# tusen-ai/RangeDet

Measured on AMD Instinct MI355X. Metric: range-image frames/sec (64x2650, 8ch) at 1/2/4/8 GPU; Meta-Kernel HBM GB/s vs peak, higher is better.
Workload: dtype bf16

## Files before the change

### include/rangedet_hip.h

```cpp
#ifndef RANGEDET_HIP_H_
#define RANGEDET_HIP_H_
#include <stddef.h>
#include <stdint.h>

#ifdef __cplusplus
extern "C" {
#endif

#define RD_OK 0
#define RD_EINVAL (-1)
#define RD_ESHAPE (-2)
#define RD_EWORKSPACE (-3)
#define RD_EHIP (-4)

#define RD_F32 0
#define RD_BF16 1
#define RD_F16 2

#define RD_RELU_PRE 1
#define RD_ADD 2
#define RD_RELU_POST 4
#define RD_SCALE_FOLDED 8
#define RD_MFMA16 16

int rd_version(void);
const char* rd_last_error_string(void);

int rd_nchw_to_nhwc(const float* src, void* dst, int B, int C, int H, int W, int dst_cstride, int dst_coff,
                    int zero_pad, int dst_dtype, void* stream);
int rd_nhwc_to_nchw(const void* src, float* dst, int B, int C, int H, int W, int src_cstride, int src_coff,
                    int src_dtype, void* stream);

int rd_copy_rows(const void* src, long src_row_bytes, void* dst, long dst_row_bytes, long dst_offset_bytes, long bytes,
                 int rows, void* stream);

size_t rd_conv_packed_bytes(int ntaps, int cin, int cout, int dtype);
int rd_pack_conv_weight_host(const float* w_oihw_host, int cout, int cin, int kh, int kw, int dtype,
                             void* packed_host);
int rd_deconv_phase_taps(int kh, int kw, int stride_w, int pad_w, int phase);
int rd_pack_deconv_weight_host(const float* w_iohw_host, int cin, int cout, int kh, int kw, int stride_w,
                               int pad_w, int phase, int dtype, void* packed_host);
int rd_pack_deconv_weight_folded_host(const float* w_iohw_host, const float* fold_scale_host, int cin, int cout, int kh, int kw,
                                      int stride_w, int pad_w, int phase, int dtype, void* packed_host);

int rd_conv2d_bn_act(const void* x, int x_cstride, int x_coff, const void* w_packed, const float* scale,
                     const float* shift, const void* residual, int r_cstride, int r_coff, void* y,
                     int y_cstride, int y_coff, int B, int H, int Win, int cin, int cout, int kh, int kw,
                     int stride_w, int flags, int dtype, void* stream);
size_t rd_conv3x3_ex_packed_bytes(int cin, int cout, int stride_w, int x_cstride);
int rd_pack_conv3x3_ex_host(const float* w_oihw_host, const float* fold_scale_host, int cout, int cin, int stride_w,
                            int x_cstride, int dtype, void* packed_host);
int rd_pack_conv3x3_m16_host(const float* w_oihw_host, const float* fold_scale_host, int cout, int cin, int dtype, void* packed_host);
int rd_conv3x3_mfma16_ok(int cin, int cout, int stride_w, int W, int fused_output_conv);
size_t rd_conv1x1_sc_packed_bytes(int cin, int cout);
int rd_pack_conv1x1_sc_host(const float* w_oi_host, const float* fold_scale_host, int cout, int cin, int dtype,
                            void* packed_host);
int rd_conv3x3_bn_act_ex(const void* x, int x_cstride, int x_coff, const void* w_packed, const float* scale, const float* shift,
                         const void* residual, int r_cstride, int r_coff, const void* sc_x, int sc_cstride, int sc_coff,
                         int sc_cin, const void* sc_w_packed, void* y, int y_cstride, int y_coff, int B, int H, int Win, int cin,
                         int cout, int stride_w, int flags, int dtype, void* stream);
size_t rd_block64_packed_bytes(int cin);
int rd_pack_block64_host(const float* w1_oihw_host, const float* fold_scale1_host, const float* w2_oihw_host,
                         const float* fold_scale2_host, int cin, int dtype, void* packed_host);
int rd_block64_bn_act(const void* x, int x_cstride, int x_coff, int cin, const void* w_packed, const float* shift1, const float* shift2,
                      const void* sc_w_packed, void* y, int y_cstride, int y_coff, int B, int H, int W, int dtype, void* stream);
int rd_pack_block64_m16_host(const float* w1_oihw_host, const float* fold_scale1_host, const float* w2_oihw_host,
                             const float* fold_scale2_host, int dtype, void* packed_host);
int rd_pack_conv1x1_sc_m16_host(const float* w_oi_host, const float* fold_scale_host, int dtype, void* packed_host);
int rd_block64_m16_bn_act(const void* x, int x_cstride, int x_coff, const void* w_packed, const float* shift1, const float* shift2,
                          const void* sc_w_packed, void* y, int y_cstride, int y_coff, int B, int H, int W, int dtype, void* stream);

size_t rd_head_packed_bytes(void);
int rd_pack_head_weight_host(const float* w, int nout, int cin, int dtype, void* out_host);
size_t rd_head_m16_packed_bytes(void);
int rd_pack_head_weight_m16_host(const float* w, int nout, int cin, int dtype, void* out_host);
int rd_conv2d_bn_act_head_out(const void* x, int x_cstride, int x_coff, const void* w_packed, const float* scale,
                              const float* shift, int B, int H, int W, int cin, int flags, const void* head_w_packed,
                              const float* head_bias, float* out, long out_batch_stride, long n_off, int nout, int dtype,
                              void* stream);

int rd_conv3x3_bn_act_pair(const void* x0, int x0_coff, const void* w0_packed, const float* shift0, void* y0, int y0_coff,
                           const void* x1, int x1_coff, const void* w1_packed, const float* shift1, void* y1, int y1_coff,
                           int x_cstride, int y_cstride, int B, int H, int W, int cin, int flags, int dtype, void* stream);
int rd_conv2d_bn_act_head_out_pair(const void* x0, int x0_coff, const void* w0_packed, const float* shift0, const void* head_w0_packed,
                                   const float* head_bias0, float* out0, long out0_batch_stride, int nout0,
                                   const void* x1, int x1_coff, const void* w1_packed, const float* shift1, const void* head_w1_packed,
                                   const float* head_bias1, float* out1, long out1_batch_stride, int nout1,
                                   int x_cstride, long n_off, int B, int H, int W, int cin, int flags, int dtype, void* stream);

size_t rd_conv3x3_cat_packed_bytes(int cin1, int cin2, int cout);
int rd_pack_conv3x3_cat_host(const float* w, const float* fold_scale, int cout, int cin1, int cin2, int dtype, void* out_host);
int rd_conv3x3_bn_act_cat(const void* x1, int x1_cstride, int x1_coff, int cin1, const void* x2, int x2_cstride, int x2_coff, int cin2,
                          const void* w_packed, const float* shift, void* y, int y_cstride, int y_coff, int B, int H, int W, int cout,
                          int flags, int dtype, void* stream);

int rd_deconv2d_bn_act(const void* x, int x_cstride, int x_coff, const void* w_packed_phase,
                       const float* scale, const float* shift, const void* residual, int r_cstride,
                       int r_coff, void* y, int y_cstride, int y_coff, int B, int H, int Win, int cin,
                       int cout, int kh, int kw, int stride_w, int pad_w, int phase, int flags, int dtype,
                       void* stream);

int rd_deconv2d_all_phases_ok(int kh, int kw, int stride_w, int pad_w, int cout, int dtype);
int rd_deconv2d_bn_act_all(const void* x, int x_cstride, int x_coff, const void* w_packed_all, long w_phase_bytes,
                           const float* shift, const void* residual, int r_cstride, int r_coff, void* y, int y_cstride,
                           int y_coff, int B, int H, int Win, int cin, int cout, int kh, int kw, int stride_w, int pad_w,
                           int flags, int dtype, void* stream);

int rd_deconv2d_phase_pairs_ok(int kh, int kw, int stride_w, int pad_w, int cout, int dtype);
int rd_pack_deconv_phase_pair_host(const void* phase_a, const void* phase_b, int cin, int dtype, void* out);
int rd_deconv2d_bn_act_pairs(const void* x, int x_cstride, int x_coff, const void* w_packed_pairs, long w_pair_bytes,
                             const float* shift2, const void* residual, int r_cstride, int r_coff, void* y, int y_cstride,
                             int y_coff, int B, int H, int Win, int cin, int cout, int kh, int kw, int stride_w, int pad_w,
                             int flags, int dtype, void* stream);

int rd_head_out(const void* x, int x_cstride, int x_coff, const float* w, const float* bias, float* out,
                long out_batch_stride, long n_off, int B, int H, int W, int cin, int nout, int dtype,
                void* stream);

size_t rd_meta_packed_bytes(int dtype);
int rd_pack_meta_host(const float* w0, const float* b0, const float* w1, const float* b1, const float* s1,
                      const float* t1, const float* agg, const float* s2, const float* t2, int dtype,
                      void* packed_host);
int rd_meta_kernel_fwd(const void* data, int d_cstride, int d_coff, const float* coord_nchw,
                       const void* packed, void* y, int y_cstride, int y_coff, int B, int H, int W, int dtype,
                       void* stream);

size_t rd_sorted_foreground_workspace_bytes(long N, long k);
int rd_sorted_foreground(const float* cls_score, const float* bbox_delta, const float* pc, const float* mask,
                         int B, long N, long k, int D, int apply_sigmoid, float* out_score, float* out_delta,
                         float* out_pc, int* out_idx, void* ws, size_t ws_bytes, void* stream);

int rd_decode3d_bbox(const float* bbox_delta, const float* pc, float* out, int B, long N, int box_type,
                     int is_bin, void* stream);

size_t rd_score_filter_workspace_bytes(long n);
int rd_score_filter_dets(const float* scores, const float* boxes10, long n, float min_score, float* dets,
                         int* d_count, void* ws, size_t ws_bytes, void* stream);
int rd_score_filter_dets_batched(const float* scores, long scores_bstride, const float* boxes10, long boxes_bstride,
                                 long n, float min_score, float* dets, long dets_bstride, int* d_count, void* ws,
                                 size_t ws_bytes, int B, void* stream);

#define RD_WNMS_MAX_K 65536
#define RD_TIE_STABLE 0
#define RD_TIE_REFERENCE 1
#define RD_WNMS_DIAG_NO_SKIP 0x100
#define RD_WNMS_DIAG_TILE_W(n) (((n) & 0xff) << 16)
#define RD_WNMS_DIAG_MERGE_LDS(n) (((n) & 0x7f) << 24)
size_t rd_wnms_workspace_bytes(int Kcap);
int rd_wnms_4c(const float* dets, int Kcap, const int* d_count, const int* order, int tie_order, float thresh,
               float thresh_vote, int is3d, int hash_scale, float* out_dets, int* keep, int* d_nkeep, void* ws,
               size_t ws_bytes, void* stream);
int rd_wnms_4c_batched(const float* dets, long dets_bstride, int Kcap, const int* d_count, const int* order,
                       long order_bstride, int tie_order, float thresh, float thresh_vote, int is3d, int hash_scale,
                       float* out_dets, long out_bstride, int* keep, long keep_bstride, int* d_nkeep, void* ws,
                       size_t ws_bytes, int B, void* stream);
int rd_single_overlap(const float* dets_a, const float* dets_b, long n, int is3d, float* out, void* stream);
int rd_wnms_pair_skippable(const float* dets_a, const float* dets_b, long n, unsigned char* out, void* stream);

int rd_edge_atan2f(const float* y, const float* x, long n, float* out, void* stream);

int rd_wnms_order_host(const float* dets_host, int K, int* order_host);

int rd_dets12_to_8(const float* dets12, int Mcap, const int* d_count, float* out8, void* stream);
int rd_dets12_to_8_batched(const float* dets12, long dets12_bstride, int Mcap, const int* d_count, float* out8,
                           long out8_bstride, int B, void* stream);

int rd_rotated_iou_8pt(const float* boxes1, const float* boxes2, float* ious, long n1, long n2, void* stream);
int rd_batch_rotated_iou(const float* proposal, int p_stride, const float* gt_bbox, float* iou_map, int* argmax, int B, long N,
                         int n_gt, void* stream);
int rd_batch_rotated_iou_3d(const float* proposal, int p_stride, const float* gt_bbox7, float* iou_map, int* argmax, int B, long N,
                            int n_gt, void* stream);
int rd_rotated_iou_7(const float* boxes1, const float* boxes2, float* ious, long n1, long n2, void* stream);
int rd_batch_max_iou(const float* proposals, int p_stride, const float* gt8, float* out, long n, int n_gt,
                     void* stream);

size_t rd_nms3d_workspace_bytes(long N, int B);
int rd_gather_keep_scores(const float* score, long score_bstride, int k, const int* keep_idx, int max_keep, float* out, int B,
                          void* stream);
int rd_nms3d(const float* boxes, int B, long N, float iou_thres, int max_keep, int normal_iou, int* keep_idx,
             float* bbox_after_nms, void* ws, size_t ws_bytes, void* stream);

int rd_assign3d_v2(const float* pc, const float* bbox, const float* bbox_center, const float* bbox_radius, const float* mask,
                   const float* is_in_nlz, long N, int M, float max_x, float min_x, float max_y, float min_y, float max_z,
                   float min_z, float max_dist, int* out, void* stream);
size_t rd_get_point_num_workspace_bytes(void);
int rd_get_point_num(const float* bbox_inds, long N, float* out, void* ws, size_t ws_bytes, void* stream);

typedef struct {
  float clip_lo[7], clip_hi[7];
  float mean[8], sd[8];
  float interval_lo[3], interval_hi[3];
} rd_input_norm_t;
int rd_input_transform(const float* range_image, const float* pc_vehicle_frame, const float* inclination,
                       const rd_input_norm_t* norm_host, int B, int H, int W, int Hp, int Wp, float* input_data,
                       float* coord_s1, float* pc_s1, float* pc_s2, float* pc_s4, float* mask_s1, float* mask_s2,
                       float* mask_s4, void* stream);

typedef struct {
  float *input_data, *coord_s1;
  float *pc[3], *mask[3];
  float *reg_target[3], *reg_weight[3], *reg_normalize_weight[3], *cls_target[3];
  int* bbox3d_ind;
} rd_train_outputs_t;
size_t rd_train_transform_workspace_bytes(int B);
int rd_train_transform(const float* range_image, const float* pc_vehicle_frame, const float* inclination,
                       const rd_input_norm_t* norm_host, const float* gt_bbox_imu, const float* gt_bbox_center,
                       const float* gt_limits, const float* gt_bbox_csa, const int* num_gt_host, int Mmax, float radius,
                       float max_dist, const float* reg_weight_host, int B, int H, int W, int Hp, int Wp,
                       const rd_train_outputs_t* out_host, void* ws, size_t ws_bytes, void* stream);

#define RD_PROF_CONV 0
#define RD_PROF_META 1
#define RD_PROF_HEAD_OUT 2
#define RD_PROF_SORT 3
#define RD_PROF_DECODE 4
#define RD_PROF_WNMS 5
#define RD_PROF_LAYOUT 6
#define RD_PROF_CONV3 7
#define RD_PROF_BLOCK 8
#define RD_PROF_NKINDS 9
int rd_prof_enable(int on);
int rd_prof_reset(void);
int rd_prof_get(int kind, double* total_ms, long* launches);

#ifdef __cplusplus
}
#endif
#endif
```

### rangedet_amd/csrc/k_misc.h

```cpp
#pragma once
#include "rd_common.h"

namespace rd {

template <int DT>
__global__ __launch_bounds__(256) void nchw_to_nhwc_kernel(const float* __restrict__ src, void* __restrict__ dst_, int C,
                                                           long HW, int cs, int coff, int cpad, long total) {
  using E = Elem<DT>;
  typename E::T* dst = (typename E::T*)dst_;
  const int ctot = C + cpad;
  for (long i = blockIdx.x * 256L + threadIdx.x; i < total; i += (long)gridDim.x * 256) {
    long p = i % HW;
    long rest = i / HW;
    int c = (int)(rest % ctot);
    long b = rest / ctot;
    float v = c < C ? src[(b * C + c) * HW + p] : 0.f;
    dst[(b * HW + p) * cs + coff + c] = E::from_f32(v);
  }
}
template <int DT, int NSLOT>
__global__ __launch_bounds__(256) void nchw_to_nhwc_px_kernel(const float* __restrict__ src, void* __restrict__ dst_, int C,
                                                              long HW, int cs, int coff, long npix) {
  using E = Elem<DT>;
  typename E::T* dst = (typename E::T*)dst_;
  for (long i = blockIdx.x * 256L + threadIdx.x; i < npix; i += (long)gridDim.x * 256) {
    const long b = i / HW, p = i - b * HW;
    typename E::T v[NSLOT * E::CH];
#pragma unroll
    for (int c = 0; c < NSLOT * E::CH; ++c) v[c] = E::from_f32(c < C ? src[(b * C + c) * HW + p] : 0.f);
    Slot16 pk[NSLOT];
    memcpy(pk, v, sizeof(pk));
#pragma unroll
    for (int u = 0; u < NSLOT; ++u) *(Slot16*)(dst + i * cs + coff + u * E::CH) = pk[u];
  }
}
template <int DT>
__global__ __launch_bounds__(256) void nhwc_to_nchw_kernel(const void* __restrict__ src_, float* __restrict__ dst, int C,
                                                           long HW, int cs, int coff, long total) {
  using E = Elem<DT>;
  const typename E::T* src = (const typename E::T*)src_;
  for (long i = blockIdx.x * 256L + threadIdx.x; i < total; i += (long)gridDim.x * 256) {
    long p = i % HW;
    long rest = i / HW;
    int c = (int)(rest % C);
    long b = rest / C;
    dst[(b * C + c) * HW + p] = E::to_f32(src[(b * HW + p) * cs + coff + c]);
  }
}

template <int DT, int NOUT>
__global__ __launch_bounds__(256) void head_out_kernel(const void* __restrict__ x_, int cs, int coff,
                                                       const float* __restrict__ w, const float* __restrict__ bias,
                                                       float* __restrict__ out, long out_bs, long n_off, long HW,
                                                       int cin) {
  using E = Elem<DT>;
  using T = typename E::T;
  __shared__ float wl[8 * 128];
  const T* x = (const T*)x_ + (size_t)blockIdx.y * HW * cs;
  for (int i = threadIdx.x; i < NOUT * cin; i += 256) wl[i] = w[i];
  __syncthreads();
  const int sub = threadIdx.x & 7;
  const int per = cin >> 3;
  const long npix_iter = (long)gridDim.x * 32;
  for (long p0 = blockIdx.x * 32L; p0 < HW; p0 += npix_iter) {
    long p = p0 + (threadIdx.x >> 3);
    float acc[NOUT];
#pragma unroll
    for (int o = 0; o < NOUT; ++o) acc[o] = 0.f;
    if (p < HW) {
      const T* px = x + p * cs + coff + sub * per;
      if ((per % E::CH) == 0) {
        for (int c0 = 0; c0 < per; c0 += E::CH) {
          const Slot16 raw = *(const Slot16*)(px + c0);
          T el[E::CH];
          memcpy(el, &raw, 16);
#pragma unroll
          for (int e = 0; e < E::CH; ++e) {
            const float v = E::to_f32(el[e]);
#pragma unroll
            for (int o = 0; o < NOUT; ++o) acc[o] += v * wl[o * cin + sub * per + c0 + e];
          }
        }
      } else {
        for (int c = 0; c < per; ++c) {
          float v = E::to_f32(px[c]);
#pragma unroll
          for (int o = 0; o < NOUT; ++o) acc[o] += v * wl[o * cin + sub * per + c];
        }
      }
    }
#pragma unroll
    for (int o = 0; o < NOUT; ++o) {
      acc[o] += __shfl_xor(acc[o], 1);
      acc[o] += __shfl_xor(acc[o], 2);
      acc[o] += __shfl_xor(acc[o], 4);
    }
    if (p < HW && sub == 0) {
      float* o_ = out + (size_t)blockIdx.y * out_bs + (n_off + p) * NOUT;
#pragma unroll
      for (int o = 0; o < NOUT; ++o) o_[o] = acc[o] + bias[o];
    }
  }
}

template <int NOUT, int DT = RD_BF16>
__global__ __launch_bounds__(256) void head_out_mfma_kernel(const bf16_t* __restrict__ x, int cs, int coff,
                                                            const float* __restrict__ w, const float* __restrict__ bias,
                                                            float* __restrict__ out, long out_bs, long n_off, long HW,
                                                            int cin) {
  __shared__ __attribute__((aligned(16))) unsigned char lds[4 * 8192];
  const int lane = threadIdx.x & 63, m = lane & 31, hi = lane >> 5, wv = threadIdx.x >> 6;
  unsigned char* img = lds + wv * 8192;
  const int nks = cin >> 4, nsl = cin >> 3;
  x += (size_t)blockIdx.y * HW * cs + coff;
  out += (size_t)blockIdx.y * out_bs + n_off * NOUT;
  s16x8 wh[8], wl[8];
#pragma unroll
  for (int ks = 0; ks < 8; ++ks) {
    unsigned short h[8], l[8];
#pragma unroll
    for (int j = 0; j < 8; ++j) {
      const float v = (m < NOUT && ks < nks) ? w[m * cin + ks * 16 + hi * 8 + j] : 0.f;
      h[j] = H16<DT>::from_f32(v);
      l[j] = H16<DT>::from_f32(v - H16<DT>::to_f32(h[j]));
    }
    memcpy(&wh[ks], h, 16);
    memcpy(&wl[ks], l, 16);
  }
  float bs[4];
#pragma unroll
  for (int r = 0; r < 4; ++r) bs[r] = 4 * hi + r < NOUT ? bias[4 * hi + r] : 0.f;
  const long ntile = (HW + 31) / 32;
  const long wave0 = (long)blockIdx.x * 4 + wv, nwave = (long)gridDim.x * 4;
  const int lp = lane >> 4, ls = lane & 15;
  auto load = [&](long tile, Slot16 (&v)[8]) {
#pragma unroll
    for (int it = 0; it < 8; ++it) {
      const long p = min(tile * 32 + it * 4 + lp, HW - 1);
      v[it] = ls < nsl ? *(const Slot16*)(x + p * cs + ls * 8) : Slot16{0u, 0u, 0u, 0u};
    }
  };
  Slot16 cur[8], nxt[8];
  if (wave0 < ntile) load(wave0, cur);
  for (long tile = wave0; tile < ntile; tile += nwave) {
    const bool more = tile + nwave < ntile;
    if (more) load(tile + nwave, nxt);
#pragma unroll
    for (int it = 0; it < 8; ++it) {
      const int pr = it * 4 + lp;
      *(Slot16*)(img + pr * 256 + ((ls ^ (pr & 15)) << 4)) = cur[it];
    }
    __builtin_amdgcn_wave_barrier();
    f32x16 acc;
#pragma unroll
    for (int r = 0; r < 16; ++r) acc[r] = 0.f;
#pragma unroll
    for (int ks = 0; ks < 8; ++ks) {
      const s16x8 b = *(const s16x8*)(img + m * 256 + (((2 * ks + hi) ^ (m & 15)) << 4));
      acc = H16<DT>::mfma(wl[ks], b, acc);
      acc = H16<DT>::mfma(wh[ks], b, acc);
    }
    __builtin_amdgcn_wave_barrier();
    const long p = tile * 32 + m;
    if (p < HW) {
      float* o = out + p * NOUT + 4 * hi;
#pragma unroll
      for (int r = 0; r < 4; ++r)
        if (4 * hi + r < NOUT) o[r] = acc[r] + bs[r];
    }
    if (more) {
#pragma unroll
      for (int it = 0; it < 8; ++it) cur[it] = nxt[it];
    }
  }
}

__global__ __launch_bounds__(256) void decode3d_kernel(const float* __restrict__ delta, const float* __restrict__ pc,
                                                       float* __restrict__ out, long n, int box_type, int is_bin) {
  long idx = blockIdx.x * 256L + threadIdx.x;
  if (idx >= n) return;
  const float* d = delta + idx * box_type;
  float pc_x = pc[idx * 3 + 0], pc_y = pc[idx * 3 + 1], pc_z = pc[idx * 3 + 2];
  float az = atan2f(pc_y, pc_x);
  float ca = cosf(az), sa = sinf(az);
  float dx, dy, width, length, height, z0, yaw_l;
  if (is_bin) {
    dx = d[0];
    dy = d[1];
    width = expf(d[3]);
    length = expf(d[4]);
    height = expf(d[5]);
    float cz = pc_z + d[2];
    z0 = (float)((double)cz - (double)height / 2.0);
    yaw_l = d[6] + az;
  } else {
    dx = d[0] * fabsf(d[0]);
    dy = d[1] * fabsf(d[1]);
    width = expf(d[2]);
    length = expf(d[3]);
    height = expf(d[7]);
    z0 = d[6];
    yaw_l = atan2f(d[5], d[4]) + az;
  }
  float dxl = dx * ca - dy * sa;
  float dyl = dx * sa + dy * ca;
  float cx = pc_x + dxl, cy = pc_y + dyl;
  float sy = sinf(yaw_l), cyw = cosf(yaw_l);
  float hl = (float)(0.5 * (double)length), hw = (float)(0.5 * (double)width);
  float hx[4] = {hl, -hl, -hl, hl};
  float hy[4] = {-hw, -hw, hw, hw};
  float* o = out + idx * 10;
#pragma unroll
  for (int k = 0; k < 4; ++k) {
    o[2 * k] = (hx[k] * cyw - hy[k] * sy) + cx;
    o[2 * k + 1] = (hx[k] * sy + hy[k] * cyw) + cy;
  }
  o[8] = z0;
  o[9] = z0 + height;
}

__global__ __launch_bounds__(256) void filter_count_kernel(const float* __restrict__ scores, long n, float thr,
                                                           int* __restrict__ blk_cnt, long sc_bs, long blk_bs) {
  scores += blockIdx.y * sc_bs;
  blk_cnt += blockIdx.y * blk_bs;
  long i = blockIdx.x * 256L + threadIdx.x;
  int p = (i < n) && (scores[i] > thr);
  unsigned long long m = __ballot(p);
  __shared__ int wc[4];
  if ((threadIdx.x & 63) == 0) wc[threadIdx.x >> 6] = __popcll(m);
  __syncthreads();
  if (threadIdx.x == 0) blk_cnt[blockIdx.x] = wc[0] + wc[1] + wc[2] + wc[3];
}
__global__ __launch_bounds__(256) void filter_scan_kernel(int* __restrict__ blk_cnt, int nblk, int* __restrict__ total,
                                                          long blk_bs) {
  blk_cnt += blockIdx.x * blk_bs;
  total += blockIdx.x;
  __shared__ int part[256];
  __shared__ int carry;
  if (threadIdx.x == 0) carry = 0;
  __syncthreads();
  for (int base = 0; base < nblk; base += 256) {
    int i = base + threadIdx.x;
    int v = i < nblk ? blk_cnt[i] : 0;
    part[threadIdx.x] = v;
    __syncthreads();
    for (int off = 1; off < 256; off <<= 1) {
      int t = threadIdx.x >= off ? part[threadIdx.x - off] : 0;
      __syncthreads();
      part[threadIdx.x] += t;
      __syncthreads();
    }
    int incl = part[threadIdx.x];
    if (i < nblk) blk_cnt[i] = carry + incl - v;
    __syncthreads();
    if (threadIdx.x == 255) carry += incl;
    __syncthreads();
  }
  if (threadIdx.x == 0) *total = carry;
}
__global__ __launch_bounds__(256) void filter_scatter_kernel(const float* __restrict__ scores,
                                                             const float* __restrict__ boxes10, long n, float thr,
                                                             const int* __restrict__ blk_off, float* __restrict__ dets,
                                                             long sc_bs, long box_bs, long blk_bs, long dets_bs) {
  scores += blockIdx.y * sc_bs;
  boxes10 += blockIdx.y * box_bs;
  blk_off += blockIdx.y * blk_bs;
  dets += blockIdx.y * dets_bs;
  long i = blockIdx.x * 256L + threadIdx.x;
  int p = (i < n) && (scores[i] > thr);
  unsigned long long m = __ballot(p);
  __shared__ int wc[4];
  const int wv = threadIdx.x >> 6, ln = threadIdx.x & 63;
  if (ln == 0) wc[wv] = __popcll(m);
  __syncthreads();
  int off = blk_off[blockIdx.x];
  for (int w = 0; w < wv; ++w) off += wc[w];
  if (p) {
    int pos = off + __popcll(m & ((1ull << ln) - 1ull));
    const float* b = boxes10 + i * 10;
    float* d = dets + (size_t)pos * 12;
#pragma unroll
    for (int k = 0; k < 8; ++k) d[k] = b[k];
    d[8] = fdlibm_atan2f(b[1] - b[3], b[0] - b[2]);
    d[9] = b[8];
    d[10] = b[9] - b[8];
    d[11] = scores[i];
  }
}

__global__ __launch_bounds__(256) void dets12_to_8_kernel(const float* __restrict__ d12, int cap, const int* __restrict__ d_count,
                                                          float* __restrict__ o8, long d12_bs, long o8_bs) {
  d12 += blockIdx.y * d12_bs;
  o8 += blockIdx.y * o8_bs;
  int i = blockIdx.x * 256 + threadIdx.x;
  int n = d_count ? min(d_count[blockIdx.y], cap) : cap;
  if (i >= n) return;
  const float* d = d12 + (size_t)i * 12;
  float* o = o8 + (size_t)i * 8;
  o[0] = (d[0] + d[2] + d[4] + d[6]) / 4.f;
  o[1] = (d[1] + d[3] + d[5] + d[7]) / 4.f;
  o[2] = d[9] + d[10] / 2.f;
  float ax = d[2] - d[0], ay = d[3] - d[1];
  float bx = d[2] - d[4], by = d[3] - d[5];
  o[3] = sqrtf(ax * ax + ay * ay);
  o[4] = sqrtf(bx * bx + by * by);
  o[5] = d[10];
  o[6] = d[8];
  o[7] = d[11];
}

__global__ __launch_bounds__(256) void gather_keep_scores_kernel(const float* __restrict__ score, long score_bs, int k,
                                                                 const int* __restrict__ keep, int mk, float* __restrict__ out) {
  const int i = blockIdx.x * 256 + threadIdx.x;
  if (i >= mk) return;
  const int q = keep[(size_t)blockIdx.y * mk + i];
  out[(size_t)blockIdx.y * mk + i] = (q >= 0 && q < k) ? score[blockIdx.y * score_bs + q] : -__builtin_inff();
}

}
```

### rangedet_amd/csrc/k_sort.h

```cpp
#pragma once
#include "rd_common.h"

namespace rd {

constexpr int SORT_TILE = 2048;

__device__ __forceinline__ unsigned desc_key(float f) {
  unsigned u = __float_as_uint(f);
  unsigned asc = u ^ ((u >> 31) ? 0xFFFFFFFFu : 0x80000000u);
  return ~asc;
}
__device__ __forceinline__ float key_to_float(unsigned key) {
  unsigned asc = ~key;
  unsigned u = (asc >> 31) ? (asc ^ 0x80000000u) : ~asc;
  return __uint_as_float(u);
}

__global__ __launch_bounds__(256) void sort_keygen_kernel(const float* __restrict__ score, const float* __restrict__ mask,
                                                          long N, int apply_sigmoid, unsigned* __restrict__ keys,
                                                          unsigned* __restrict__ idx, long ws_stride) {
  long i = blockIdx.x * 256L + threadIdx.x;
  if (i >= N) return;
  const long b = blockIdx.y;
  float s = score[b * N + i];
  if (apply_sigmoid) s = 1.0f / (1.0f + expf(-s));
  if (mask) s = s * mask[b * N + i];
  keys[b * ws_stride + i] = desc_key(s);
  idx[b * ws_stride + i] = (unsigned)i;
}
__global__ __launch_bounds__(256) void sort_keygen_dets_kernel(const float* __restrict__ dets, int cap,
                                                               const int* __restrict__ d_count, unsigned* __restrict__ keys,
                                                               unsigned* __restrict__ idx) {
  int i = blockIdx.x * 256 + threadIdx.x;
  if (i >= cap) return;
  int n = d_count ? min(*d_count, cap) : cap;
  keys[i] = i < n ? desc_key(dets[(size_t)i * 12 + 11]) : 0xFFFFFFFFu;
  idx[i] = (unsigned)i;
}

__global__ __launch_bounds__(256) void sort_hist_kernel(const unsigned* __restrict__ keys, long N, int shift,
                                                        unsigned* __restrict__ hist, unsigned* __restrict__ tot,
                                                        long ws_stride, const unsigned* __restrict__ d_n) {
  if (d_n) N = min(N, (long)d_n[blockIdx.y * ws_stride]);
  keys += blockIdx.y * ws_stride;
  hist += blockIdx.y * ws_stride;
  tot += blockIdx.y * ws_stride;
  __shared__ unsigned h[256];
  h[threadIdx.x] = 0;
  __syncthreads();
  long base = (long)blockIdx.x * SORT_TILE;
  for (int r = 0; r < SORT_TILE / 256; ++r) {
    long i = base + r * 256 + threadIdx.x;
    if (i < N) atomicAdd(&h[(keys[i] >> shift) & 255u], 1u);
  }
  __syncthreads();
  unsigned v = h[threadIdx.x];
  hist[(size_t)blockIdx.x * 256 + threadIdx.x] = v;
  if (v) atomicAdd(&tot[threadIdx.x], v);
}

__global__ __launch_bounds__(256) void sort_scatter_kernel(const unsigned* __restrict__ keys_in,
                                                           const unsigned* __restrict__ idx_in, long N, int shift,
                                                           const unsigned* __restrict__ hist,
                                                           const unsigned* __restrict__ tot,
                                                           unsigned* __restrict__ keys_out, unsigned* __restrict__ idx_out,
                                                           long ws_stride, const unsigned* __restrict__ d_n) {
  if (d_n) {
    N = min(N, (long)d_n[blockIdx.y * ws_stride]);
    if ((long)blockIdx.x * SORT_TILE >= N) return;
  }
  {
    const long o = blockIdx.y * ws_stride;
    keys_in += o; idx_in += o; hist += o; tot += o; keys_out += o; idx_out += o;
  }
  __shared__ unsigned wcnt[4][256];
  __shared__ unsigned gbase[256];
  __shared__ unsigned scan[256];
  const int tid = threadIdx.x, lane = tid & 63, wv = tid >> 6;
  for (int w = 0; w < 4; ++w) wcnt[w][tid] = 0;
  {
    unsigned t = tot[tid];
    scan[tid] = t;
    __syncthreads();
    for (int off = 1; off < 256; off <<= 1) {
      unsigned a = tid >= off ? scan[tid - off] : 0u;
      __syncthreads();
      scan[tid] += a;
      __syncthreads();
    }
    unsigned before = 0;
    for (unsigned b = 0; b < blockIdx.x; ++b) before += hist[(size_t)b * 256 + tid];
    gbase[tid] = scan[tid] - t + before;
  }
  __syncthreads();

  unsigned key[8], id[8], pos[8];
  const long base = (long)blockIdx.x * SORT_TILE + wv * 512;
  const unsigned long long lt = (1ull << lane) - 1ull;
#pragma unroll
  for (int r = 0; r < 8; ++r) {
    long i = base + r * 64 + lane;
    bool valid = i < N;
    key[r] = valid ? keys_in[i] : 0xFFFFFFFFu;
    id[r] = valid ? idx_in[i] : 0u;
    unsigned d = (key[r] >> shift) & 255u;
    unsigned long long peers = __ballot(valid);
#pragma unroll
    for (int bit = 0; bit < 8; ++bit) {
      unsigned long long bm = __ballot(valid && ((d >> bit) & 1u));
      peers &= ((d >> bit) & 1u) ? bm : ~bm;
    }
    unsigned rank = __popcll(peers & lt), cnt = __popcll(peers);
    unsigned prev = wcnt[wv][d];
    pos[r] = prev + rank;
    __builtin_amdgcn_wave_barrier();
    if (valid && rank == 0) wcnt[wv][d] = prev + cnt;
    __builtin_amdgcn_wave_barrier();
  }
  __syncthreads();
  {
    unsigned c0 = wcnt[0][tid], c1 = wcnt[1][tid], c2 = wcnt[2][tid];
    wcnt[0][tid] = 0;
    wcnt[1][tid] = c0;
    wcnt[2][tid] = c0 + c1;
    wcnt[3][tid] = c0 + c1 + c2;
  }
  __syncthreads();
#pragma unroll
  for (int r = 0; r < 8; ++r) {
    long i = base + r * 64 + lane;
    if (i < N) {
      unsigned d = (key[r] >> shift) & 255u;
      unsigned dst = gbase[d] + wcnt[wv][d] + pos[r];
      keys_out[dst] = key[r];
      idx_out[dst] = id[r];
    }
  }
}

__global__ __launch_bounds__(256) void sort_gather_kernel(const unsigned* __restrict__ keys, const unsigned* __restrict__ idx,
                                                          long k, int D, const float* __restrict__ delta,
                                                          const float* __restrict__ pc, float* __restrict__ out_score,
                                                          float* __restrict__ out_delta, float* __restrict__ out_pc,
                                                          int* __restrict__ out_idx, long ws_stride, long N) {
  long i = blockIdx.x * 256L + threadIdx.x;
  if (i >= k) return;
  {
    const long b = blockIdx.y;
    keys += b * ws_stride; idx += b * ws_stride;
    delta += b * N * D; pc += b * N * 3;
    out_score += b * k; out_delta += b * k * D; out_pc += b * k * 3;
    if (out_idx) out_idx += b * k;
  }
  unsigned j = idx[i];
  out_score[i] = key_to_float(keys[i]);
  for (int c = 0; c < D; ++c) out_delta[i * D + c] = delta[(size_t)j * D + c];
  out_pc[i * 3 + 0] = pc[(size_t)j * 3 + 0];
  out_pc[i * 3 + 1] = pc[(size_t)j * 3 + 1];
  out_pc[i * 3 + 2] = pc[(size_t)j * 3 + 2];
  if (out_idx) out_idx[i] = (int)j;
}

constexpr int SEL_BINS = 4096, SEL_SHIFT = 20;
__global__ __launch_bounds__(256) void select_hist_kernel(const unsigned* __restrict__ keys, long N, unsigned* __restrict__ h12,
                                                          long ws_stride) {
  keys += blockIdx.y * ws_stride; h12 += blockIdx.y * ws_stride;
  __shared__ unsigned h[SEL_BINS];
  for (int i = threadIdx.x; i < SEL_BINS; i += 256) h[i] = 0;
  __syncthreads();
  const long base = (long)blockIdx.x * SORT_TILE;
  for (int r = 0; r < SORT_TILE / 256; ++r) {
    const long i = base + r * 256 + threadIdx.x;
    if (i < N) atomicAdd(&h[keys[i] >> SEL_SHIFT], 1u);
  }
  __syncthreads();
  for (int i = threadIdx.x; i < SEL_BINS; i += 256)
    if (h[i]) atomicAdd(&h12[i], h[i]);
}
__global__ __launch_bounds__(256) void select_thresh_kernel(const unsigned* __restrict__ h12, long k, unsigned* __restrict__ sel,
                                                            long ws_stride) {
  h12 += blockIdx.y * ws_stride; sel += blockIdx.y * ws_stride;
  __shared__ unsigned part[256];
  const int tid = threadIdx.x;
  unsigned loc[SEL_BINS / 256], sum = 0;
#pragma unroll
  for (int j = 0; j < SEL_BINS / 256; ++j) { loc[j] = h12[tid * (SEL_BINS / 256) + j]; sum += loc[j]; }
  part[tid] = sum;
  __syncthreads();
  for (int off = 1; off < 256; off <<= 1) {
    const unsigned v = tid >= off ? part[tid - off] : 0u;
    __syncthreads();
    part[tid] += v;
    __syncthreads();
  }
  unsigned before = part[tid] - sum;
  if (tid == 255 && (k == 0 || part[255] < (unsigned)k)) { sel[0] = SEL_BINS - 1; sel[1] = part[255]; }
  if (before < (unsigned)k && before + sum >= (unsigned)k) {
#pragma unroll
    for (int j = 0; j < SEL_BINS / 256; ++j) {
      if (before < (unsigned)k && before + loc[j] >= (unsigned)k) { sel[0] = tid * (SEL_BINS / 256) + j; sel[1] = before + loc[j]; }
      before += loc[j];
    }
  }
}
__global__ __launch_bounds__(256) void select_count_kernel(const unsigned* __restrict__ keys, long N, const unsigned* __restrict__ sel,
                                                           unsigned* __restrict__ cnt, long ws_stride) {
  keys += blockIdx.y * ws_stride; sel += blockIdx.y * ws_stride; cnt += blockIdx.y * ws_stride;
  const unsigned T = sel[0];
  __shared__ unsigned c;
  if (threadIdx.x == 0) c = 0;
  __syncthreads();
  const long base = (long)blockIdx.x * SORT_TILE;
  unsigned mine = 0;
  for (int r = 0; r < SORT_TILE / 256; ++r) {
    const long i = base + r * 256 + threadIdx.x;
    if (i < N && (keys[i] >> SEL_SHIFT) <= T) ++mine;
  }
  if (mine) atomicAdd(&c, mine);
  __syncthreads();
  if (threadIdx.x == 0) cnt[blockIdx.x] = c;
}
__global__ __launch_bounds__(256) void select_compact_kernel(const unsigned* __restrict__ keys_in, const unsigned* __restrict__ idx_in,
                                                             long N, const unsigned* __restrict__ sel,
                                                             const unsigned* __restrict__ cnt, unsigned* __restrict__ keys_out,
                                                             unsigned* __restrict__ idx_out, long ws_stride) {
  {
    const long o = blockIdx.y * ws_stride;
    keys_in += o; idx_in += o; sel += o; cnt += o; keys_out += o; idx_out += o;
  }
  const unsigned T = sel[0];
  __shared__ unsigned wcnt[4][8], sbase;
  const int tid = threadIdx.x, lane = tid & 63, wv = tid >> 6;
  if (tid == 0) {
    unsigned b = 0;
    for (unsigned j = 0; j < blockIdx.x; ++j) b += cnt[j];
    sbase = b;
  }
  const long base = (long)blockIdx.x * SORT_TILE + wv * 512;
  unsigned key[8], id[8];
  unsigned long long m[8];
#pragma unroll
  for (int r = 0; r < 8; ++r) {
    const long i = base + r * 64 + lane;
    const bool valid = i < N;
    key[r] = valid ? keys_in[i] : 0xFFFFFFFFu;
    id[r] = valid ? idx_in[i] : 0u;
    m[r] = __ballot(valid && (key[r] >> SEL_SHIFT) <= T);
    if (lane == 0) wcnt[wv][r] = (unsigned)__popcll(m[r]);
  }
  __syncthreads();
  unsigned off = sbase;
  for (int w = 0; w < wv; ++w)
#pragma unroll
    for (int r = 0; r < 8; ++r) off += wcnt[w][r];
#pragma unroll
  for (int r = 0; r < 8; ++r) {
    if ((m[r] >> lane) & 1ull) {
      const unsigned dst = off + (unsigned)__popcll(m[r] & ((1ull << lane) - 1ull));
      keys_out[dst] = key[r];
      idx_out[dst] = id[r];
    }
    off += (unsigned)__popcll(m[r]);
  }
}

struct SortWs {
  unsigned *keysA, *keysB, *idxA, *idxB, *hist, *tot, *h12, *cnt, *sel;
  int nblk;
};
inline size_t sort_ws_bytes(long N) {
  long nblk = (N + SORT_TILE - 1) / SORT_TILE;
  return (size_t)(4 * N + nblk * 256 + 4 * 256 + SEL_BINS + nblk + 64) * 4 + 256;
}
inline SortWs sort_ws_carve(void* ws, long N) {
  SortWs s;
  s.nblk = (int)((N + SORT_TILE - 1) / SORT_TILE);
  unsigned* p = (unsigned*)ws;
  s.keysA = p; p += N;
  s.keysB = p; p += N;
  s.idxA = p; p += N;
  s.idxB = p; p += N;
  s.hist = p; p += (size_t)s.nblk * 256;
  s.tot = p; p += 4 * 256;
  s.h12 = p; p += SEL_BINS;
  s.cnt = p; p += s.nblk;
  s.sel = p;
  return s;
}
inline int sort_clear(const SortWs& s, hipStream_t st, int nb, long ws_stride, bool with_h12) {
  const size_t bytes = (size_t)(4 * 256 + (with_h12 ? SEL_BINS : 0)) * 4;
  const hipError_t e = nb > 1 ? hipMemset2DAsync(s.tot, (size_t)ws_stride * 4, 0, bytes, nb, st) : hipMemsetAsync(s.tot, 0, bytes, st);
  return e == hipSuccess ? RD_OK : fail(RD_EHIP, "sort: memset");
}
inline int radix_sort_pairs(const SortWs& s, long N, hipStream_t st, int nb = 1, long ws_stride = 0, const unsigned* d_n = nullptr,
                            bool cleared = false) {
  if (!cleared) { int rc = sort_clear(s, st, nb, ws_stride, false); if (rc != RD_OK) return rc; }
  unsigned *ki = s.keysA, *ko = s.keysB, *ii = s.idxA, *io = s.idxB;
  for (int pass = 0; pass < 4; ++pass) {
    hipLaunchKernelGGL(sort_hist_kernel, dim3(s.nblk, nb), dim3(256), 0, st, ki, N, pass * 8, s.hist, s.tot + pass * 256,
                       ws_stride, d_n);
    hipLaunchKernelGGL(sort_scatter_kernel, dim3(s.nblk, nb), dim3(256), 0, st, ki, ii, N, pass * 8, s.hist,
                       s.tot + pass * 256, ko, io, ws_stride, d_n);
    std::swap(ki, ko);
    std::swap(ii, io);
  }
  return check_launch("radix_sort_pairs");
}

inline int radix_topk_pairs(const SortWs& s, long N, long k, hipStream_t st, int nb, long ws_stride, unsigned** rk, unsigned** ri) {
  const bool off = dev_switches().sort_no_select;
  *rk = s.keysA; *ri = s.idxA;
  RD_REQUIRE(k > 0 && k <= N, RD_ESHAPE, "top-k: k %ld of N %ld", k, N);
  if (off || 2 * k > N) return radix_sort_pairs(s, N, st, nb, ws_stride);
  { int rc = sort_clear(s, st, nb, ws_stride, true); if (rc != RD_OK) return rc; }
  hipLaunchKernelGGL(select_hist_kernel, dim3(s.nblk, nb), dim3(256), 0, st, s.keysA, N, s.h12, ws_stride);
  hipLaunchKernelGGL(select_thresh_kernel, dim3(1, nb), dim3(256), 0, st, s.h12, k, s.sel, ws_stride);
  hipLaunchKernelGGL(select_count_kernel, dim3(s.nblk, nb), dim3(256), 0, st, s.keysA, N, s.sel, s.cnt, ws_stride);
  hipLaunchKernelGGL(select_compact_kernel, dim3(s.nblk, nb), dim3(256), 0, st, s.keysA, s.idxA, N, s.sel, s.cnt, s.keysB, s.idxB,
                     ws_stride);
  SortWs v = s;
  v.keysA = s.keysB; v.keysB = s.keysA; v.idxA = s.idxB; v.idxB = s.idxA;
  *rk = s.keysB; *ri = s.idxB;
  return radix_sort_pairs(v, N, st, nb, ws_stride, s.sel + 1, true);
}

}
```

### rangedet_amd/csrc/rd_api.hip

```cpp
#include "k_conv1.h"
#include "k_block.h"
#include "k_assign.h"
#include "k_input.h"
#include "k_target.h"
#include "k_nms3d.h"
#include "k_meta.h"
#include "k_misc.h"
#include "k_riou.h"
#include "k_sort.h"
#include "k_wnms.h"

#include <algorithm>
#include <string>
#include <numeric>

using namespace rd;

namespace rd {
inline size_t align256(size_t v) { return (v + 255) & ~(size_t)255; }
inline size_t wnms_ws_bytes(int cap) {
  const size_t nw = (size_t)(cap + 63) / 64;
  return align256((size_t)cap * PREP_F * 4) + 3 * align256((size_t)cap * nw * 8) + 4 * align256((size_t)cap * 4) +
         align256(((size_t)cap + 2) * 8 + 3 * ((size_t)cap / 32 + 2) * 4) + align256(nw * 8) + 256 + align256(sort_ws_bytes(cap)) + 256;
}
// ... 478 lines not shown
}

int rd_deconv2d_all_phases_ok(int kh, int kw, int stride_w, int pad_w, int cout, int dtype) {
  if (!is_h16(dtype) || kh != 3 || stride_w < 2 || stride_w > 8 || !conv3_phases_eligible(cout, RD_SCALE_FOLDED)) return 0;
  if (kw - 2 * pad_w != stride_w) return 0;
  for (int p = 0; p < stride_w; ++p)
    if (!deconv_tap_set(deconv_taps_sorted(kh, kw, stride_w, pad_w, p))) return 0;
  return 1;
}
int rd_deconv2d_bn_act_all(const void* x, int x_cstride, int x_coff, const void* w_packed_all, long w_phase_bytes,
                           const float* shift, const void* residual, int r_cstride, int r_coff, void* y, int y_cstride,
                           int y_coff, int B, int H, int Win, int cin, int cout, int kh, int kw, int stride_w, int pad_w,
                           int flags, int dtype, void* stream) {
  RD_REQUIRE(x && w_packed_all && y, RD_EINVAL, "deconv2d_all: null pointer");
  RD_REQUIRE(is_h16(dtype), RD_EINVAL, "deconv2d_all: dtype %d (RD_BF16 or RD_F16)", dtype);
  RD_REQUIRE(flags & RD_SCALE_FOLDED, RD_EINVAL, "deconv2d_all: needs RD_SCALE_FOLDED weights (rd_pack_deconv_weight_folded_host)");
  RD_REQUIRE(!((flags & RD_ADD) && !residual), RD_EINVAL, "deconv2d_all: RD_ADD without residual");
  RD_REQUIRE(B > 0 && H > 0 && Win > 0 && cin > 0, RD_ESHAPE, "deconv2d_all: shape");
  RD_REQUIRE(y_coff >= 0 && y_coff + cout <= y_cstride, RD_ESHAPE, "deconv2d_all: y channels exceed stride");
  RD_REQUIRE(x_cstride % 8 == 0 && x_coff % 8 == 0 && x_coff + cin_slots(cin, RD_BF16) * 8 <= x_cstride, RD_ESHAPE, "deconv2d_all: x channel stride/offset");
  RD_REQUIRE(rd_deconv2d_all_phases_ok(kh, kw, stride_w, pad_w, cout, dtype), RD_ESHAPE,
             "deconv2d_all: kernel (%d,%d) stride %d pad %d cout %d is not a set of two-column 3x2 phases (use rd_deconv2d_bn_act per phase)",
             kh, kw, stride_w, pad_w, cout);
  RD_REQUIRE(w_phase_bytes >= (long)conv_packed_bytes(6, cin, cout, RD_BF16) && w_phase_bytes % 16 == 0, RD_EINVAL, "deconv2d_all: w_phase_bytes");
  allow_conv_lds();
  Conv3Phases ph;
  ph.nph = stride_w; ph.ts_mask = 0; ph.y_pc = y_cstride; ph.r_pc = r_cstride; ph.w_pb = w_phase_bytes;
  for (int p = 0; p < stride_w; ++p)
    if (deconv_tap_set(deconv_taps_sorted(kh, kw, stride_w, pad_w, p)) == 2) ph.ts_mask |= 1 << p;
  return launch_conv3(x, x_cstride, x_coff, w_packed_all, nullptr, shift, residual, r_cstride * stride_w, r_coff, y, y_cstride * stride_w,
                      y_coff, B, H, Win, cin, cout, flags, 1, (hipStream_t)stream, 3, nullptr, dtype, nullptr, &ph);
}

int rd_deconv2d_phase_pairs_ok(int kh, int kw, int stride_w, int pad_w, int cout, int dtype) {
  if (!rd_deconv2d_all_phases_ok(kh, kw, stride_w, pad_w, cout, dtype) || cout != 64 || stride_w % 2) return 0;
  if (!rd_deconv2d_all_phases_ok(kh, kw, stride_w, pad_w, 128, dtype)) return 0;
  for (int p = 0; p < stride_w; p += 2)
    if (deconv_tap_set(deconv_taps_sorted(kh, kw, stride_w, pad_w, p)) != deconv_tap_set(deconv_taps_sorted(kh, kw, stride_w, pad_w, p + 1))) return 0;
  return 1;
}
int rd_pack_deconv_phase_pair_host(const void* phase_a, const void* phase_b, int cin, int dtype, void* out) {
  RD_REQUIRE(phase_a && phase_b && out, RD_EINVAL, "pack_deconv_pair: null pointer");
  RD_REQUIRE(is_h16(dtype) && cin > 0, RD_EINVAL, "pack_deconv_pair: dtype %d / cin %d", dtype, cin);
  const size_t body = conv_packed_body_bytes(6, cin, 64, RD_BF16), blocks = body / 2048;
  for (size_t i = 0; i < blocks; ++i) {
    memcpy((unsigned char*)out + i * 4096, (const unsigned char*)phase_a + i * 2048, 2048);
    memcpy((unsigned char*)out + i * 4096 + 2048, (const unsigned char*)phase_b + i * 2048, 2048);
  }
  memset((unsigned char*)out + 2 * body, 0, 2 * RD_CONV_TAIL);
  return RD_OK;
}
int rd_deconv2d_bn_act_pairs(const void* x, int x_cstride, int x_coff, const void* w_packed_pairs, long w_pair_bytes,
                             const float* shift2, const void* residual, int r_cstride, int r_coff, void* y, int y_cstride,
                             int y_coff, int B, int H, int Win, int cin, int cout, int kh, int kw, int stride_w, int pad_w,
                             int flags, int dtype, void* stream) {
  RD_REQUIRE(x && w_packed_pairs && y && shift2, RD_EINVAL, "deconv2d_pairs: null pointer");
  RD_REQUIRE(is_h16(dtype), RD_EINVAL, "deconv2d_pairs: dtype %d (RD_BF16 or RD_F16)", dtype);
  RD_REQUIRE(flags & RD_SCALE_FOLDED, RD_EINVAL, "deconv2d_pairs: needs RD_SCALE_FOLDED weights (rd_pack_deconv_weight_folded_host)");
  RD_REQUIRE(!((flags & RD_ADD) && !residual), RD_EINVAL, "deconv2d_pairs: RD_ADD without residual");
  RD_REQUIRE(B > 0 && H > 0 && Win > 0 && cin > 0, RD_ESHAPE, "deconv2d_pairs: shape");
  RD_REQUIRE(x_cstride % 8 == 0 && x_coff % 8 == 0 && x_coff + cin_slots(cin, RD_BF16) * 8 <= x_cstride, RD_ESHAPE, "deconv2d_pairs: x channel stride/offset");
  RD_REQUIRE(rd_deconv2d_phase_pairs_ok(kh, kw, stride_w, pad_w, cout, dtype), RD_ESHAPE,
             "deconv2d_pairs: kernel (%d,%d) stride %d pad %d cout %d has no phase pairs (use rd_deconv2d_bn_act_all)", kh, kw, stride_w, pad_w, cout);
  RD_REQUIRE(y_cstride == cout && y_coff == 0 && (!residual || (r_cstride == cout && r_coff == 0)), RD_ESHAPE,
             "deconv2d_pairs: the output / residual must be dense %d-channel tensors (two phases are one 128-channel write)", cout);
  RD_REQUIRE(w_pair_bytes >= (long)conv_packed_bytes(6, cin, 2 * cout, RD_BF16) && w_pair_bytes % 16 == 0, RD_EINVAL, "deconv2d_pairs: w_pair_bytes");
  allow_conv_lds();
  Conv3Phases ph;
  ph.nph = stride_w / 2; ph.ts_mask = 0; ph.y_pc = 2 * cout; ph.r_pc = 2 * cout; ph.w_pb = w_pair_bytes;
  for (int p = 0; p < stride_w; p += 2)
    if (deconv_tap_set(deconv_taps_sorted(kh, kw, stride_w, pad_w, p)) == 2) ph.ts_mask |= 1 << (p / 2);
  return launch_conv3(x, x_cstride, x_coff, w_packed_pairs, nullptr, shift2, residual, r_cstride * stride_w, r_coff, y, y_cstride * stride_w,
                      y_coff, B, H, Win, cin, 2 * cout, flags, 1, (hipStream_t)stream, 3, nullptr, dtype, nullptr, &ph);
}

int rd_head_out(const void* x, int x_cstride, int x_coff, const float* w, const float* bias, float* out,
                long out_batch_stride, long n_off, int B, int H, int W, int cin, int nout, int dtype, void* stream) {
  RD_REQUIRE(x && w && bias && out, RD_EINVAL, "head_out: null pointer");
  RD_REQUIRE(cin % 8 == 0 && cin <= 128 && cin > 0, RD_ESHAPE, "head_out: cin %d (multiple of 8, <= 128)", cin);
  RD_REQUIRE(nout == 1 || nout == 7 || nout == 8, RD_ESHAPE, "head_out: nout %d not in {1,7,8}", nout);
  RD_REQUIRE(dtype == RD_F32 || is_h16(dtype), RD_EINVAL, "head_out: dtype");
  hipStream_t st = (hipStream_t)stream;
  const long HW = (long)H * W;
  dim3 grid((unsigned)std::min<long>((HW + 31) / 32, 4096), B);
  ProfScope ps(RD_PROF_HEAD_OUT, st);
  if (is_h16(dtype) && nout > 1 && cin % 16 == 0 && x_cstride % 8 == 0 && x_coff % 8 == 0) {
    dim3 g2((unsigned)std::min<long>((HW + 127) / 128, 2048), B);
#define RD_HOM(NO, DT_) hipLaunchKernelGGL((head_out_mfma_kernel<NO, DT_>), g2, dim3(256), 0, st, (const bf16_t*)x, x_cstride, x_coff, w, bias, out, out_batch_stride, n_off, HW, cin)
    if (dtype == RD_F16) { if (nout == 7) RD_HOM(7, RD_F16); else RD_HOM(8, RD_F16); }
    else { if (nout == 7) RD_HOM(7, RD_BF16); else RD_HOM(8, RD_BF16); }
#undef RD_HOM
    return check_launch("head_out");
  }
#define RD_HO(DT, NO) hipLaunchKernelGGL((head_out_kernel<DT, NO>), grid, dim3(256), 0, st, x, x_cstride, x_coff, w, bias, out, out_batch_stride, n_off, HW, cin)
  if (dtype == RD_BF16) { if (nout == 1) RD_HO(RD_BF16, 1); else if (nout == 7) RD_HO(RD_BF16, 7); else RD_HO(RD_BF16, 8); }
  else if (dtype == RD_F16) { if (nout == 1) RD_HO(RD_F16, 1); else if (nout == 7) RD_HO(RD_F16, 7); else RD_HO(RD_F16, 8); }
  else { if (nout == 1) RD_HO(RD_F32, 1); else if (nout == 7) RD_HO(RD_F32, 7); else RD_HO(RD_F32, 8); }
#undef RD_HO
  return check_launch("head_out");
}

size_t rd_meta_packed_bytes(int dtype) { return meta_layout(dtype).total; }
int rd_pack_meta_host(const float* w0, const float* b0, const float* w1, const float* b1, const float* s1,
                      const float* t1, const float* agg, const float* s2, const float* t2, int dtype, void* out) {
  RD_REQUIRE(w0 && b0 && w1 && b1 && s1 && t1 && agg && s2 && t2 && out, RD_EINVAL, "pack_meta: null pointer");
  RD_REQUIRE(dtype == RD_F32 || is_h16(dtype), RD_EINVAL, "pack_meta: dtype");
  pack_meta(w0, b0, w1, b1, s1, t1, agg, s2, t2, dtype, out);
  return RD_OK;
}
int rd_meta_kernel_fwd(const void* data, int d_cstride, int d_coff, const float* coord_nchw, const void* packed,
                       void* y, int y_cstride, int y_coff, int B, int H, int W, int dtype, void* stream) {
  RD_REQUIRE(data && coord_nchw && packed && y, RD_EINVAL, "meta_kernel: null pointer");
  RD_REQUIRE(B > 0 && H > 0 && W > 0, RD_ESHAPE, "meta_kernel: empty shape");
  RD_REQUIRE(dtype == RD_F32 || is_h16(dtype), RD_EINVAL, "meta_kernel: dtype");
  const int ch = ch_per_slot(dtype);
  RD_REQUIRE(d_cstride % ch == 0 && d_coff % ch == 0 && y_cstride % ch == 0 && y_coff % ch == 0, RD_ESHAPE,
             "meta_kernel: channel strides/offsets must be 16-byte multiples");
  RD_REQUIRE(d_coff + 64 <= d_cstride && y_coff + 64 <= y_cstride, RD_ESHAPE, "meta_kernel: needs 64 channels");
  hipStream_t st = (hipStream_t)stream;
  MetaArgs a;
  a.data = data; a.d_cs = d_cstride; a.d_co = d_coff; a.coord = coord_nchw; a.packed = (const unsigned char*)packed;
  a.y = y; a.y_cs = y_cstride; a.y_co = y_coff; a.B = B; a.H = H; a.W = W;
  constexpr int WAVES = 8;
  a.tiles_h = (H + WAVES - 1) / WAVES;
  a.tiles_w = (W + 31) / 32;
  a.ntiles = B * a.tiles_h * a.tiles_w;
  a.r0 = 0; a.m0 = a.m1 = a.m2 = 0;
  const size_t consts = 9 * 64 * 4 * 2 + 1024;
  ProfScope ps(RD_PROF_META, st);
  if (is_h16(dtype)) {
    const size_t lds = meta_layout(dtype).wbytes + consts + (size_t)(WAVES + 2) * 34 * 128 + 4096;
    static std::atomic<unsigned long long> seen{0};
    once_per_device(seen, [] { allow_big_lds(meta16_kernel<WAVES, RD_BF16>); allow_big_lds(meta16_kernel<WAVES, RD_F16>); });
    const dim3 mgrid(std::min(a.ntiles, conv_num_cus())), mblock(WAVES * 64);
    const int strips = a.tiles_w * B;
    a.r0 = dev_switches().conv_xcd && strips % 8 == 0 ? 8 : strips;
    RD_REQUIRE((unsigned long long)a.ntiles * (unsigned)std::max(a.r0, std::max(a.tiles_h, a.tiles_w)) < (1ull << 32), RD_ESHAPE,
               "meta_kernel: %d tiles exceed the range of the tile decode", a.ntiles);
    a.m0 = meta_magic(a.r0); a.m1 = meta_magic(a.tiles_h); a.m2 = meta_magic(a.tiles_w);
    RD_REQUIRE((long)H * W < (1l << 23) && (long)H * W * d_cstride < (1l << 31) && W < (1 << 23) && d_cstride < (1 << 23), RD_ESHAPE,
               "meta_kernel: image of %d x %d pixels x %d channels exceeds the 32-bit halo offsets", H, W, d_cstride);
    if (dtype == RD_F16) hipLaunchKernelGGL((meta16_kernel<WAVES, RD_F16>), mgrid, mblock, lds, st, a);
    else hipLaunchKernelGGL((meta16_kernel<WAVES, RD_BF16>), mgrid, mblock, lds, st, a);
  } else {
    const size_t lds = consts + (size_t)(WAVES + 2) * 34 * 256;
    static std::atomic<unsigned long long> seen32{0};
    once_per_device(seen32, [] { allow_big_lds(meta_kernel<RD_F32, WAVES>); });
    hipLaunchKernelGGL((meta_kernel<RD_F32, WAVES>), dim3(std::min(a.ntiles, 512)), dim3(WAVES * 64), lds, st, a);
  }
  return check_launch("meta_kernel");
}

size_t rd_sorted_foreground_workspace_bytes(long N, long k) { (void)k; return (sort_ws_bytes(N) + 256 + 255) & ~(size_t)255; }
int rd_sorted_foreground(const float* cls_score, const float* bbox_delta, const float* pc, const float* mask, int B,
                         long N, long k, int D, int apply_sigmoid, float* out_score, float* out_delta, float* out_pc,
                         int* out_idx, void* ws, size_t ws_bytes, void* stream) {
  RD_REQUIRE(cls_score && bbox_delta && pc && out_score && out_delta && out_pc && ws, RD_EINVAL, "sorted_foreground: null pointer");
  RD_REQUIRE(B > 0 && N > 0 && k > 0 && D > 0, RD_ESHAPE, "sorted_foreground: empty shape");
  RD_REQUIRE(N >= k, RD_ESHAPE, "sorted_foreground: N (%ld) < num_fgs (%ld)", N, k);
  RD_REQUIRE(N < (1L << 31), RD_ESHAPE, "sorted_foreground: N too large");
  RD_REQUIRE(ws_bytes >= rd_sorted_foreground_workspace_bytes(N, k), RD_EWORKSPACE, "sorted_foreground: workspace %zu < %zu",
             ws_bytes, rd_sorted_foreground_workspace_bytes(N, k));
  hipStream_t st = (hipStream_t)stream;
  void* wsa = (void*)(((uintptr_t)ws + 255) & ~(uintptr_t)255);
  SortWs s = sort_ws_carve(wsa, N);
  ProfScope ps(RD_PROF_SORT, st);
  const size_t per = rd_sorted_foreground_workspace_bytes(N, k);
  const bool wide = ws_bytes >= per * (size_t)B;
  const long stride = wide ? (long)(per / 4) : 0;
  const int nb = wide ? B : 1;
  for (int b0 = 0; b0 < B; b0 += nb) {
    hipLaunchKernelGGL(sort_keygen_kernel, dim3((unsigned)((N + 255) / 256), nb), dim3(256), 0, st, cls_score + (size_t)b0 * N,
                       mask ? mask + (size_t)b0 * N : nullptr, N, apply_sigmoid, s.keysA, s.idxA, stride);
    unsigned *rk, *ri;
    int rc = radix_topk_pairs(s, N, k, st, nb, stride, &rk, &ri);
    if (rc != RD_OK) return rc;
    hipLaunchKernelGGL(sort_gather_kernel, dim3((unsigned)((k + 255) / 256), nb), dim3(256), 0, st, rk, ri, k, D,
                       bbox_delta + (size_t)b0 * N * D, pc + (size_t)b0 * N * 3, out_score + (size_t)b0 * k,
                       out_delta + (size_t)b0 * k * D, out_pc + (size_t)b0 * k * 3, out_idx ? out_idx + (size_t)b0 * k : nullptr,
                       stride, N);
  }
  return check_launch("sorted_foreground");
}

int rd_decode3d_bbox(const float* bbox_delta, const float* pc, float* out, int B, long N, int box_type, int is_bin,
                     void* stream) {
  RD_REQUIRE(bbox_delta && pc && out, RD_EINVAL, "decode3d: null pointer");
  RD_REQUIRE(B > 0 && N > 0, RD_ESHAPE, "decode3d: empty shape");
  RD_REQUIRE((is_bin && box_type == 7) || (!is_bin && box_type == 8), RD_ESHAPE,
             "decode3d: box_type %d with is_bin=%d (8 for regular, 7 for bin)", box_type, is_bin);
  hipStream_t st = (hipStream_t)stream;
  const long n = (long)B * N;
  ProfScope ps(RD_PROF_DECODE, st);
  hipLaunchKernelGGL(decode3d_kernel, dim3((unsigned)((n + 255) / 256)), dim3(256), 0, st, bbox_delta, pc, out, n, box_type, is_bin);
  return check_launch("decode3d");
}

size_t rd_score_filter_workspace_bytes(long n) { return (size_t)((n + 255) / 256 + 8) * 4 + 256; }
int rd_score_filter_dets_batched(const float* scores, long scores_bstride, const float* boxes10, long boxes_bstride,
                                 long n, float min_score, float* dets, long dets_bstride, int* d_count, void* ws,
                                 size_t ws_bytes, int B, void* stream) {
  RD_REQUIRE(scores && boxes10 && dets && d_count && ws, RD_EINVAL, "score_filter: null pointer");
  RD_REQUIRE(n > 0 && B > 0, RD_ESHAPE, "score_filter: empty input");
  const size_t per = rd_score_filter_workspace_bytes(n);
  RD_REQUIRE(ws_bytes >= per * (size_t)B, RD_EWORKSPACE, "score_filter: workspace %zu < %zu", ws_bytes, per * (size_t)B);
  hipStream_t st = (hipStream_t)stream;
  int* blk = (int*)(((uintptr_t)ws + 255) & ~(uintptr_t)255);
  const int nblk = (int)((n + 255) / 256);
  const long blk_bs = nblk + 8;
  ProfScope ps(RD_PROF_WNMS, st);
  hipLaunchKernelGGL(filter_count_kernel, dim3(nblk, B), dim3(256), 0, st, scores, n, min_score, blk, scores_bstride, blk_bs);
  hipLaunchKernelGGL(filter_scan_kernel, dim3(B), dim3(256), 0, st, blk, nblk, d_count, blk_bs);
  hipLaunchKernelGGL(filter_scatter_kernel, dim3(nblk, B), dim3(256), 0, st, scores, boxes10, n, min_score, blk, dets,
                     scores_bstride, boxes_bstride, blk_bs, dets_bstride);
  return check_launch("score_filter");
}
int rd_score_filter_dets(const float* scores, const float* boxes10, long n, float min_score, float* dets, int* d_count,
                         void* ws, size_t ws_bytes, void* stream) {
  return rd_score_filter_dets_batched(scores, 0, boxes10, 0, n, min_score, dets, 0, d_count, ws, ws_bytes, 1, stream);
}

size_t rd_wnms_workspace_bytes(int Kcap) { return Kcap > 0 ? wnms_ws_bytes(Kcap) : 0; }
int rd_wnms_4c_batched(const float* dets, long dets_bstride, int Kcap, const int* d_count, const int* order,
                       long order_bstride, int tie_order, float thresh, float thresh_vote, int is3d, int hash_scale,
                       float* out_dets, long out_bstride, int* keep, long keep_bstride, int* d_nkeep, void* ws,
                       size_t ws_bytes, int B, void* stream) {
  RD_REQUIRE(dets && out_dets && keep && d_nkeep && ws, RD_EINVAL, "wnms_4c: null pointer");
  RD_REQUIRE(Kcap > 0 && Kcap <= RD_WNMS_MAX_K, RD_ESHAPE, "wnms_4c: Kcap %d not in [1, %d]", Kcap, RD_WNMS_MAX_K);
  RD_REQUIRE(B > 0, RD_ESHAPE, "wnms_4c: batch %d", B);
  const int diag = tie_order & ~0xff;
  tie_order &= 0xff;
  RD_REQUIRE(tie_order == RD_TIE_STABLE || tie_order == RD_TIE_REFERENCE, RD_EINVAL, "wnms_4c: tie_order %d", tie_order);
  RD_REQUIRE(!(diag & ~(RD_WNMS_DIAG_NO_SKIP | (0xff << 16) | (0x7f << 24))), RD_EINVAL, "wnms_4c: unknown diagnostic bits 0x%x", diag);
  const size_t per = rd_wnms_workspace_bytes(Kcap);
  RD_REQUIRE(ws_bytes >= per * (size_t)B, RD_EWORKSPACE, "wnms_4c: workspace %zu < %zu", ws_bytes, per * (size_t)B);
  RD_REQUIRE(order || B == 1 || tie_order == RD_TIE_REFERENCE, RD_EINVAL,
             "wnms_4c: the batched call needs an explicit processing order or RD_TIE_REFERENCE");
  hipStream_t st = (hipStream_t)stream;
  static std::atomic<unsigned long long> seen_lds{0};
  once_per_device(seen_lds, [] {
    allow_big_lds(wnms_tie_order_kernel); allow_big_lds(wnms_scan_kernel); allow_big_lds(wnms_scan4_kernel); allow_big_lds(wnms_merge_kernel);
  });
  WnmsWs w = wnms_ws_carve(ws, Kcap);
  ProfScope ps(RD_PROF_WNMS, st);
  WnmsBatch bs;
  bs.dets = dets_bstride; bs.order = order_bstride; bs.prep = (long)(per / 4); bs.words = (long)(per / 8);
  bs.ints = (long)(per / 4); bs.keep = keep_bstride; bs.out = out_bstride;
  const int* ord = order;
  if (!ord && tie_order == RD_TIE_REFERENCE) {
    const size_t lds = TIE_STACK_BYTES + (Kcap <= TIE_LDS_K ? (size_t)Kcap * 8 + 3 * ((size_t)Kcap / 32 + 2) * 4 : 0);
    hipLaunchKernelGGL(wnms_tie_order_kernel, dim3(1, 1, B), dim3(256), lds, st, dets, Kcap, d_count, w.order, bs, (long)(per / 4),
                       w.scratch);
    ord = w.order;
    bs.order = (long)(per / 4);
  } else if (!ord) {
    void* swa = (void*)(((uintptr_t)w.sort_ws + 255) & ~(uintptr_t)255);
    SortWs s = sort_ws_carve(swa, Kcap);
    hipLaunchKernelGGL(sort_keygen_dets_kernel, dim3((Kcap + 255) / 256), dim3(256), 0, st, dets, Kcap, d_count, s.keysA, s.idxA);
    int rc = radix_sort_pairs(s, Kcap, st);
    if (rc != RD_OK) return rc;
    if (hipMemcpyAsync(w.order, s.idxA, (size_t)Kcap * 4, hipMemcpyDeviceToDevice, st) != hipSuccess)
      return rd::fail(RD_EHIP, "wnms_4c: order copy");
    ord = w.order;
    bs.order = 0;
  }
  const int nb = (Kcap + 63) / 64;
  hipLaunchKernelGGL(wnms_prep_kernel, dim3((Kcap + 255) / 256, 1, B), dim3(256), 0, st, dets, ord, Kcap, d_count, w.prep, bs,
                     (float)hash_scale, w.novf);
  const int e_tw = (diag >> 16) & 0xff, e_ml = (diag >> 24) & 0x7f;
  const int tile_w = std::min(w.nwcap, e_tw ? std::max(1, e_tw) : 256);
  const size_t scan_lds = ((size_t)w.nwcap + (size_t)64 * tile_w) * 8;
  const int R1 = 256, nb1 = R1 / 64;
  const bool one_round = dev_switches().wnms_one_round;
  const bool two = Kcap >= 4 * R1 && !one_round;
  const int ct = dev_switches().wnms_ct == 32 ? 32 : dev_switches().wnms_ct == 16 ? 16 : 8;
  const int pgrid = std::min(2048, std::max(64, nb * (64 / ct) * std::min(nb, 16)));
  const int allow_skip = thresh >= 1e-3f && thresh_vote >= 1e-3f && !is3d && !dev_switches().wnms_no_skip && !(diag & RD_WNMS_DIAG_NO_SKIP);
  auto pairs = [&](const int* rows, const int* nrows, const unsigned long long* supp, int rb_end) {
    auto k = dev_switches().wnms_bal ? (ct == 8 ? wnms_pairs_kernel<8, true> : ct == 16 ? wnms_pairs_kernel<16, true> : wnms_pairs_kernel<32, true>)
                                     : (ct == 8 ? wnms_pairs_kernel<8, false> : ct == 16 ? wnms_pairs_kernel<16, false> : wnms_pairs_kernel<32, false>);
    hipLaunchKernelGGL(k, dim3(pgrid, 1, B), dim3(64), 0, st, w.prep, Kcap, d_count, thresh, thresh_vote, is3d, w.thr, w.vote,
                       w.nwcap, bs, rows, nrows, supp, 0, rb_end, allow_skip);
  };
  pairs(nullptr, nullptr, nullptr, two ? nb1 : nb);
  const bool scan4 = w.nwcap <= 128 && !e_tw && !dev_switches().wnms_scan1;
  const int tile_words = 64 * 128;
  const size_t scan4_lds = ((size_t)w.nwcap + tile_words) * 8;
  auto scan = [&](int c_begin, int c_end, unsigned long long* state) {
    if (scan4)
      hipLaunchKernelGGL(wnms_scan4_kernel, dim3(1, 1, B), dim3(256), scan4_lds, st, w.thr, w.snap, Kcap, d_count, w.nwcap, ord,
                         w.keep_q, keep, d_nkeep, bs, c_begin, c_end, state, tile_words);
    else
      hipLaunchKernelGGL(wnms_scan_kernel, dim3(1, 1, B), dim3(64), scan_lds, st, w.thr, w.snap, Kcap, d_count, w.nwcap, ord,
                         w.keep_q, keep, d_nkeep, bs, c_begin, c_end, state, tile_w);
  };
  scan(0, two ? nb1 : nb, two ? w.supp_state : (unsigned long long*)nullptr);
  if (two) {
    hipLaunchKernelGGL(wnms_alive_kernel, dim3(1, 1, B), dim3(256), 0, st, w.supp_state, Kcap, d_count, R1, w.alive, w.nalive, bs);
    pairs((const int*)w.alive, (const int*)w.nalive, (const unsigned long long*)w.supp_state, 0);
    scan(nb1, nb, w.supp_state);
  }
  const int lds_cap = std::min(Kcap + 2, e_ml ? std::max(4, e_ml) : 2048);
  hipLaunchKernelGGL(wnms_merge_kernel, dim3(std::min(Kcap, 4096), 1, B), dim3(64), (size_t)lds_cap * 8, st, dets, ord, w.vote,
                     w.snap, Kcap, d_count, w.nwcap, w.keep_q, d_nkeep, out_dets, bs, lds_cap, w.ovf, w.novf);
  if (Kcap + 2 > lds_cap)
    hipLaunchKernelGGL(wnms_merge_big_kernel, dim3(1, 1, B), dim3(64), 0, st, dets, ord, w.vote, w.snap, Kcap, d_count, w.nwcap,
                       w.keep_q, out_dets, bs, (const int*)w.ovf, (const int*)w.novf, w.scratch);
  return check_launch("wnms_4c");
}
int rd_wnms_4c(const float* dets, int Kcap, const int* d_count, const int* order, int tie_order, float thresh,
               float thresh_vote, int is3d, int hash_scale, float* out_dets, int* keep, int* d_nkeep, void* ws,
               size_t ws_bytes, void* stream) {
  return rd_wnms_4c_batched(dets, 0, Kcap, d_count, order, 0, tie_order, thresh, thresh_vote, is3d, hash_scale, out_dets, 0,
                            keep, 0, d_nkeep, ws, ws_bytes, 1, stream);
}
int rd_single_overlap(const float* dets_a, const float* dets_b, long n, int is3d, float* out, void* stream) {
  RD_REQUIRE(n >= 0 && (n == 0 || (dets_a && dets_b && out)), RD_EINVAL, "single_overlap: bad arguments");
  if (n == 0) return RD_OK;
  hipLaunchKernelGGL(single_overlap_kernel, dim3((unsigned)((n + 63) / 64)), dim3(64), 0, (hipStream_t)stream, dets_a, dets_b, n,
                     is3d, out);
  return check_launch("single_overlap");
}
int rd_wnms_pair_skippable(const float* dets_a, const float* dets_b, long n, unsigned char* out, void* stream) {
  RD_REQUIRE(dets_a && dets_b && out && n >= 0, RD_EINVAL, "wnms_pair_skippable: null pointer");
  if (n == 0) return RD_OK;
  hipLaunchKernelGGL(pair_skippable_kernel, dim3((unsigned)((n + 63) / 64)), dim3(64), 0, (hipStream_t)stream, dets_a, dets_b, n, out);
  return check_launch("wnms_pair_skippable");
}
namespace rd {
__global__ void atan2f_kernel(const float* y, const float* x, long n, float* out) {
  const long i = (long)blockIdx.x * blockDim.x + threadIdx.x;
  if (i < n) out[i] = fdlibm_atan2f(y[i], x[i]);
}
}
int rd_edge_atan2f(const float* y, const float* x, long n, float* out, void* stream) {
  RD_REQUIRE(y && x && out && n >= 0, RD_EINVAL, "edge_atan2f: null pointer");
  if (n == 0) return RD_OK;
  hipLaunchKernelGGL(atan2f_kernel, dim3((unsigned)((n + 255) / 256)), dim3(256), 0, (hipStream_t)stream, y, x, n, out);
  return check_launch("edge_atan2f");
}
int rd_wnms_order_host(const float* dets_host, int K, int* order_host) {
  RD_REQUIRE(K >= 0 && (K == 0 || (dets_host && order_host)), RD_EINVAL, "wnms_order_host: bad arguments");
  std::iota(order_host, order_host + K, 0);
  std::sort(order_host, order_host + K, [&](int i, int j) { return dets_host[i * 12 + 11] > dets_host[j * 12 + 11]; });
  return RD_OK;
}

int rd_dets12_to_8_batched(const float* dets12, long dets12_bstride, int Mcap, const int* d_count, float* out8,
                           long out8_bstride, int B, void* stream) {
  RD_REQUIRE(dets12 && out8, RD_EINVAL, "dets12_to_8: null pointer");
  RD_REQUIRE(Mcap > 0 && B > 0, RD_ESHAPE, "dets12_to_8: empty input");
  hipLaunchKernelGGL(dets12_to_8_kernel, dim3((Mcap + 255) / 256, B), dim3(256), 0, (hipStream_t)stream, dets12, Mcap, d_count,
                     out8, dets12_bstride, out8_bstride);
  return check_launch("dets12_to_8");
}
int rd_dets12_to_8(const float* dets12, int Mcap, const int* d_count, float* out8, void* stream) {
  return rd_dets12_to_8_batched(dets12, 0, Mcap, d_count, out8, 0, 1, stream);
}

int rd_gather_keep_scores(const float* score, long score_bstride, int k, const int* keep_idx, int max_keep, float* out, int B,
                          void* stream) {
  RD_REQUIRE(score && keep_idx && out, RD_EINVAL, "gather_keep_scores: null pointer");
  RD_REQUIRE(k > 0 && max_keep > 0 && B > 0, RD_ESHAPE, "gather_keep_scores: empty input");
  hipLaunchKernelGGL(gather_keep_scores_kernel, dim3((max_keep + 255) / 256, B), dim3(256), 0, (hipStream_t)stream, score,
                     score_bstride, k, keep_idx, max_keep, out);
  return check_launch("gather_keep_scores");
}

// ... 188 lines not shown
```

### rangedet_amd/lib.py

```python
import ctypes
import os

import numpy as np

RD_OK, RD_EINVAL, RD_ESHAPE, RD_EWORKSPACE, RD_EHIP = 0, -1, -2, -3, -4
RD_F32, RD_BF16, RD_F16 = 0, 1, 2
H16 = (RD_BF16, RD_F16)
RD_RELU_PRE, RD_ADD, RD_RELU_POST, RD_SCALE_FOLDED, RD_MFMA16 = 1, 2, 4, 8, 16
RD_WNMS_MAX_K = 65536
RD_WNMS_DIAG_NO_SKIP = 0x100


def RD_WNMS_DIAG_TILE_W(n):
    return (n & 0xff) << 16


def RD_WNMS_DIAG_MERGE_LDS(n):
    return (n & 0x7f) << 24

RD_TIE_STABLE, RD_TIE_REFERENCE = 0, 1
PROF_KINDS = {"conv": 0, "meta": 1, "head_out": 2, "sort": 3, "decode": 4, "wnms": 5, "layout": 6, "conv3": 7, "block": 8}

_HERE = os.path.dirname(os.path.abspath(__file__))
DEFAULT_PATH = os.environ.get("RANGEDET_HIP_LIB") or os.path.join(_HERE, "librangedet_hip.so")

c_int, c_long, c_float, c_size_t, c_void_p = ctypes.c_int, ctypes.c_long, ctypes.c_float, ctypes.c_size_t, ctypes.c_void_p

SIGNATURES = {
    "rd_version": (c_int, []),
    "rd_last_error_string": (ctypes.c_char_p, []),
    "rd_nchw_to_nhwc": (c_int, [c_void_p, c_void_p, c_int, c_int, c_int, c_int, c_int, c_int, c_int, c_int, c_void_p]),
    "rd_nhwc_to_nchw": (c_int, [c_void_p, c_void_p, c_int, c_int, c_int, c_int, c_int, c_int, c_int, c_void_p]),
    "rd_copy_rows": (c_int, [c_void_p, c_long, c_void_p, c_long, c_long, c_long, c_int, c_void_p]),
    "rd_conv_packed_bytes": (c_size_t, [c_int, c_int, c_int, c_int]),
    "rd_pack_conv_weight_host": (c_int, [c_void_p, c_int, c_int, c_int, c_int, c_int, c_void_p]),
    "rd_deconv_phase_taps": (c_int, [c_int, c_int, c_int, c_int, c_int]),
    "rd_pack_deconv_weight_host": (c_int, [c_void_p, c_int, c_int, c_int, c_int, c_int, c_int, c_int, c_int, c_void_p]),
    "rd_pack_deconv_weight_folded_host": (c_int, [c_void_p, c_void_p, c_int, c_int, c_int, c_int, c_int, c_int, c_int, c_int, c_void_p]),
    "rd_conv2d_bn_act": (c_int, [c_void_p, c_int, c_int, c_void_p, c_void_p, c_void_p, c_void_p, c_int, c_int, c_void_p,
                                 c_int, c_int, c_int, c_int, c_int, c_int, c_int, c_int, c_int, c_int, c_int, c_int, c_void_p]),
    "rd_conv3x3_ex_packed_bytes": (c_size_t, [c_int, c_int, c_int, c_int]),
    "rd_pack_conv3x3_ex_host": (c_int, [c_void_p, c_void_p, c_int, c_int, c_int, c_int, c_int, c_void_p]),
    "rd_pack_conv3x3_m16_host": (c_int, [c_void_p, c_void_p, c_int, c_int, c_int, c_void_p]),
    "rd_conv3x3_mfma16_ok": (c_int, [c_int, c_int, c_int, c_int, c_int]),
    "rd_conv1x1_sc_packed_bytes": (c_size_t, [c_int, c_int]),
    "rd_pack_conv1x1_sc_host": (c_int, [c_void_p, c_void_p, c_int, c_int, c_int, c_void_p]),
    "rd_conv3x3_bn_act_ex": (c_int, [c_void_p, c_int, c_int, c_void_p, c_void_p, c_void_p, c_void_p, c_int, c_int, c_void_p, c_int,
                                     c_int, c_int, c_void_p, c_void_p, c_int, c_int, c_int, c_int, c_int, c_int, c_int, c_int,
                                     c_int, c_int, c_void_p]),
    "rd_deconv2d_bn_act": (c_int, [c_void_p, c_int, c_int, c_void_p, c_void_p, c_void_p, c_void_p, c_int, c_int, c_void_p,
                                   c_int, c_int, c_int, c_int, c_int, c_int, c_int, c_int, c_int, c_int, c_int, c_int,
                                   c_int, c_int, c_void_p]),
    "rd_conv3x3_cat_packed_bytes": (c_size_t, [c_int, c_int, c_int]),
    "rd_pack_conv3x3_cat_host": (c_int, [c_void_p, c_void_p, c_int, c_int, c_int, c_int, c_void_p]),
    "rd_conv3x3_bn_act_cat": (c_int, [c_void_p, c_int, c_int, c_int, c_void_p, c_int, c_int, c_int, c_void_p, c_void_p, c_void_p, c_int, c_int,
                                      c_int, c_int, c_int, c_int, c_int, c_int, c_void_p]),
    "rd_deconv2d_all_phases_ok": (c_int, [c_int, c_int, c_int, c_int, c_int, c_int]),
    "rd_deconv2d_bn_act_all": (c_int, [c_void_p, c_int, c_int, c_void_p, c_long, c_void_p, c_void_p, c_int, c_int, c_void_p,
                                       c_int, c_int, c_int, c_int, c_int, c_int, c_int, c_int, c_int, c_int, c_int, c_int,
                                       c_int, c_void_p]),
    "rd_deconv2d_phase_pairs_ok": (c_int, [c_int, c_int, c_int, c_int, c_int, c_int]),
    "rd_pack_deconv_phase_pair_host": (c_int, [c_void_p, c_void_p, c_int, c_int, c_void_p]),
    "rd_deconv2d_bn_act_pairs": (c_int, [c_void_p, c_int, c_int, c_void_p, c_long, c_void_p, c_void_p, c_int, c_int, c_void_p,
                                         c_int, c_int, c_int, c_int, c_int, c_int, c_int, c_int, c_int, c_int, c_int, c_int,
                                         c_int, c_void_p]),
    "rd_block64_packed_bytes": (c_size_t, [c_int]),
    "rd_pack_block64_host": (c_int, [c_void_p, c_void_p, c_void_p, c_void_p, c_int, c_int, c_void_p]),
    "rd_pack_block64_m16_host": (c_int, [c_void_p, c_void_p, c_void_p, c_void_p, c_int, c_void_p]),
    "rd_pack_conv1x1_sc_m16_host": (c_int, [c_void_p, c_void_p, c_int, c_void_p]),
    "rd_block64_m16_bn_act": (c_int, [c_void_p, c_int, c_int, c_void_p, c_void_p, c_void_p, c_void_p, c_void_p, c_int, c_int, c_int, c_int,
                                      c_int, c_int, c_void_p]),
    "rd_block64_bn_act": (c_int, [c_void_p, c_int, c_int, c_int, c_void_p, c_void_p, c_void_p, c_void_p, c_void_p, c_int, c_int, c_int, c_int,
                                  c_int, c_int, c_void_p]),
    "rd_head_packed_bytes": (c_size_t, []),
    "rd_head_m16_packed_bytes": (c_size_t, []),
    "rd_pack_head_weight_host": (c_int, [c_void_p, c_int, c_int, c_int, c_void_p]),
    "rd_pack_head_weight_m16_host": (c_int, [c_void_p, c_int, c_int, c_int, c_void_p]),
    "rd_conv2d_bn_act_head_out": (c_int, [c_void_p, c_int, c_int, c_void_p, c_void_p, c_void_p, c_int, c_int, c_int, c_int, c_int,
                                          c_void_p, c_void_p, c_void_p, c_long, c_long, c_int, c_int, c_void_p]),
    "rd_conv3x3_bn_act_pair": (c_int, [c_void_p, c_int, c_void_p, c_void_p, c_void_p, c_int] * 2 +
                               [c_int, c_int, c_int, c_int, c_int, c_int, c_int, c_int, c_void_p]),
    "rd_conv2d_bn_act_head_out_pair": (c_int, [c_void_p, c_int, c_void_p, c_void_p, c_void_p, c_void_p, c_void_p, c_long, c_int] * 2 +
                                       [c_int, c_long, c_int, c_int, c_int, c_int, c_int, c_int, c_void_p]),
    "rd_head_out": (c_int, [c_void_p, c_int, c_int, c_void_p, c_void_p, c_void_p, c_long, c_long, c_int, c_int, c_int,
                            c_int, c_int, c_int, c_void_p]),
    "rd_meta_packed_bytes": (c_size_t, [c_int]),
    "rd_pack_meta_host": (c_int, [c_void_p] * 9 + [c_int, c_void_p]),
    "rd_meta_kernel_fwd": (c_int, [c_void_p, c_int, c_int, c_void_p, c_void_p, c_void_p, c_int, c_int, c_int, c_int,
                                   c_int, c_int, c_void_p]),
    "rd_sorted_foreground_workspace_bytes": (c_size_t, [c_long, c_long]),
    "rd_sorted_foreground": (c_int, [c_void_p, c_void_p, c_void_p, c_void_p, c_int, c_long, c_long, c_int, c_int,
                                     c_void_p, c_void_p, c_void_p, c_void_p, c_void_p, c_size_t, c_void_p]),
    "rd_decode3d_bbox": (c_int, [c_void_p, c_void_p, c_void_p, c_int, c_long, c_int, c_int, c_void_p]),
    "rd_score_filter_workspace_bytes": (c_size_t, [c_long]),
    "rd_score_filter_dets": (c_int, [c_void_p, c_void_p, c_long, c_float, c_void_p, c_void_p, c_void_p, c_size_t, c_void_p]),
    "rd_score_filter_dets_batched": (c_int, [c_void_p, c_long, c_void_p, c_long, c_long, c_float, c_void_p, c_long, c_void_p,
                                             c_void_p, c_size_t, c_int, c_void_p]),
    "rd_wnms_workspace_bytes": (c_size_t, [c_int]),
    "rd_wnms_4c_batched": (c_int, [c_void_p, c_long, c_int, c_void_p, c_void_p, c_long, c_int, c_float, c_float, c_int, c_int,
                                   c_void_p, c_long, c_void_p, c_long, c_void_p, c_void_p, c_size_t, c_int, c_void_p]),
    "rd_dets12_to_8_batched": (c_int, [c_void_p, c_long, c_int, c_void_p, c_void_p, c_long, c_int, c_void_p]),
    "rd_wnms_4c": (c_int, [c_void_p, c_int, c_void_p, c_void_p, c_int, c_float, c_float, c_int, c_int, c_void_p, c_void_p,
                           c_void_p, c_void_p, c_size_t, c_void_p]),
    "rd_single_overlap": (c_int, [c_void_p, c_void_p, c_long, c_int, c_void_p, c_void_p]),
    "rd_wnms_order_host": (c_int, [c_void_p, c_int, c_void_p]),
    "rd_edge_atan2f": (c_int, [c_void_p, c_void_p, c_long, c_void_p, c_void_p]),
    "rd_wnms_pair_skippable": (c_int, [c_void_p, c_void_p, c_long, c_void_p, c_void_p]),
    "rd_dets12_to_8": (c_int, [c_void_p, c_int, c_void_p, c_void_p, c_void_p]),
    "rd_rotated_iou_8pt": (c_int, [c_void_p, c_void_p, c_void_p, c_long, c_long, c_void_p]),
    "rd_batch_rotated_iou": (c_int, [c_void_p, c_int, c_void_p, c_void_p, c_void_p, c_int, c_long, c_int, c_void_p]),
    "rd_batch_rotated_iou_3d": (c_int, [c_void_p, c_int, c_void_p, c_void_p, c_void_p, c_int, c_long, c_int, c_void_p]),
    "rd_rotated_iou_7": (c_int, [c_void_p, c_void_p, c_void_p, c_long, c_long, c_void_p]),
    "rd_batch_max_iou": (c_int, [c_void_p, c_int, c_void_p, c_void_p, c_long, c_int, c_void_p]),
    "rd_gather_keep_scores": (c_int, [c_void_p, c_long, c_int, c_void_p, c_int, c_void_p, c_int, c_void_p]),
    "rd_nms3d_workspace_bytes": (c_size_t, [c_long, c_int]),
    "rd_nms3d": (c_int, [c_void_p, c_int, c_long, c_float, c_int, c_int, c_void_p, c_void_p, c_void_p, c_size_t, c_void_p]),
    "rd_assign3d_v2": (c_int, [c_void_p] * 6 + [c_long, c_int] + [c_float] * 7 + [c_void_p, c_void_p]),
    "rd_get_point_num_workspace_bytes": (c_size_t, []),
    "rd_get_point_num": (c_int, [c_void_p, c_long, c_void_p, c_void_p, c_size_t, c_void_p]),
    "rd_input_transform": (c_int, [c_void_p, c_void_p, c_void_p, c_void_p, c_int, c_int, c_int, c_int, c_int] + [c_void_p] * 8 + [c_void_p]),
    "rd_train_transform_workspace_bytes": (c_size_t, [c_int]),
    "rd_train_transform": (c_int, [c_void_p] * 9 + [c_int, c_float, c_float, c_void_p, c_int, c_int, c_int, c_int, c_int,
                                   c_void_p, c_void_p, c_size_t, c_void_p]),
    "rd_prof_enable": (c_int, [c_int]),
    "rd_prof_reset": (c_int, []),
    "rd_prof_get": (c_int, [c_int, ctypes.POINTER(ctypes.c_double), ctypes.POINTER(c_long)]),
}


class RangeDetError(RuntimeError):
    def __init__(self, code, msg):
        super().__init__("librangedet_hip error %d: %s" % (code, msg))
        self.code = code


def ptr(x):
    if x is None:
        return None
    if isinstance(x, int):
        return x
    if isinstance(x, np.ndarray):
        return x.ctypes.data
    if hasattr(x, "data_ptr"):
        return x.data_ptr()
    raise TypeError("cannot take the address of %r" % type(x))


class Lib:
    def __init__(self, path=DEFAULT_PATH):
        if not os.path.exists(path):
            raise RuntimeError(
                "%s not found: the HIP extension is not built (run `python -m rangedet_amd.build`). "
                "There is no CPU fallback." % path)
        self.path = path
        if os.path.basename(path).startswith("librangedet_hip"):
            try:
                import torch
            except ImportError:
                pass
        self.cdll = ctypes.CDLL(path)
        for name, (res, args) in SIGNATURES.items():
            fn = getattr(self.cdll, name)
            fn.restype = res
            fn.argtypes = args
        self.rd_last_error_string = self.cdll.rd_last_error_string

    def call(self, name, *args):
        rc = getattr(self.cdll, name)(*args)
        if rc < 0:
            raise RangeDetError(rc, self.cdll.rd_last_error_string().decode())
        return rc

    def raw(self, name):
        return getattr(self.cdll, name)

    def pack_conv_weight(self, w_oihw, dtype):
        w = np.ascontiguousarray(w_oihw, dtype=np.float32)
        cout, cin, kh, kw = w.shape
        out = np.zeros(self.cdll.rd_conv_packed_bytes(kh * kw, cin, cout, dtype), dtype=np.uint8)
        self.call("rd_pack_conv_weight_host", w.ctypes.data, cout, cin, kh, kw, dtype, out.ctypes.data)
        return out

    def pack_conv3x3_ex(self, w_oihw, stride_w, x_cstride, fold_scale=None, dtype=RD_BF16):
        w = np.ascontiguousarray(w_oihw, dtype=np.float32)
        cout, cin = w.shape[:2]
        assert w.shape[2:] == (3, 3)
        fs = None if fold_scale is None else np.ascontiguousarray(fold_scale, dtype=np.float32)
        out = np.zeros(self.cdll.rd_conv3x3_ex_packed_bytes(cin, cout, stride_w, x_cstride), dtype=np.uint8)
        self.call("rd_pack_conv3x3_ex_host", w.ctypes.data, None if fs is None else fs.ctypes.data, cout, cin, stride_w,
                  x_cstride, dtype, out.ctypes.data)
        return out

    def pack_conv3x3_m16(self, w_oihw, fold_scale, dtype=RD_BF16):
        w = np.ascontiguousarray(w_oihw, dtype=np.float32)
        cout, cin = w.shape[:2]
        assert w.shape[2:] == (3, 3)
        fs = np.ascontiguousarray(fold_scale, dtype=np.float32)
        out = np.zeros(self.cdll.rd_conv3x3_ex_packed_bytes(cin, cout, 1, cin), dtype=np.uint8)
        self.call("rd_pack_conv3x3_m16_host", w.ctypes.data, fs.ctypes.data, cout, cin, dtype, out.ctypes.data)
        return out

    def pack_conv3x3_cat(self, w_oihw, cin1, cin2, fold_scale=None, dtype=RD_BF16):
        w = np.ascontiguousarray(w_oihw, dtype=np.float32)
        cout = w.shape[0]
        assert w.shape[1:] == (cin1 + cin2, 3, 3)
        fs = None if fold_scale is None else np.ascontiguousarray(fold_scale, dtype=np.float32)
        out = np.zeros(self.cdll.rd_conv3x3_cat_packed_bytes(cin1, cin2, cout), dtype=np.uint8)
        self.call("rd_pack_conv3x3_cat_host", w.ctypes.data, None if fs is None else fs.ctypes.data, cout, cin1, cin2, dtype, out.ctypes.data)
        return out

    def pack_conv1x1_sc(self, w_oi, fold_scale=None, dtype=RD_BF16):
        w = np.ascontiguousarray(w_oi, dtype=np.float32).reshape(w_oi.shape[0], -1)
        cout, cin = w.shape
        fs = None if fold_scale is None else np.ascontiguousarray(fold_scale, dtype=np.float32)
        out = np.zeros(self.cdll.rd_conv1x1_sc_packed_bytes(cin, cout), dtype=np.uint8)
        self.call("rd_pack_conv1x1_sc_host", w.ctypes.data, None if fs is None else fs.ctypes.data, cout, cin, dtype, out.ctypes.data)
        return out

    def pack_block64(self, w1_oihw, scale1, w2_oihw, scale2, dtype=RD_BF16, m16=False):
        w1, w2 = (np.ascontiguousarray(w, dtype=np.float32) for w in (w1_oihw, w2_oihw))
        s1, s2 = (np.ascontiguousarray(v, dtype=np.float32) for v in (scale1, scale2))
        cin = w1.shape[1]
        assert w1.shape == (64, cin, 3, 3) and w2.shape == (64, 64, 3, 3) and s1.shape == (64,) and s2.shape == (64,)
        out = np.zeros(self.cdll.rd_block64_packed_bytes(cin), dtype=np.uint8)
        if m16:
            assert cin == 64
            self.call("rd_pack_block64_m16_host", w1.ctypes.data, s1.ctypes.data, w2.ctypes.data, s2.ctypes.data, dtype, out.ctypes.data)
        else:
            self.call("rd_pack_block64_host", w1.ctypes.data, s1.ctypes.data, w2.ctypes.data, s2.ctypes.data, cin, dtype, out.ctypes.data)
        return out

    def pack_conv1x1_sc_m16(self, w_oi, fold_scale, dtype=RD_BF16):
        w = np.ascontiguousarray(w_oi, dtype=np.float32).reshape(64, 64)
        fs = np.ascontiguousarray(fold_scale, dtype=np.float32)
        out = np.zeros(self.cdll.rd_conv1x1_sc_packed_bytes(64, 64), dtype=np.uint8)
        self.call("rd_pack_conv1x1_sc_m16_host", w.ctypes.data, fs.ctypes.data, dtype, out.ctypes.data)
        return out

    def pack_deconv_weight(self, w_iohw, stride_w, pad_w, phase, dtype, fold_scale=None):
        w = np.ascontiguousarray(w_iohw, dtype=np.float32)
        cin, cout, kh, kw = w.shape
        nt = self.cdll.rd_deconv_phase_taps(kh, kw, stride_w, pad_w, phase)
        if nt < 0:
            raise RangeDetError(nt, "deconv phase taps")
        out = np.zeros(self.cdll.rd_conv_packed_bytes(nt, cin, cout, dtype), dtype=np.uint8)
        fs = None if fold_scale is None else np.ascontiguousarray(fold_scale, dtype=np.float32)
        self.call("rd_pack_deconv_weight_folded_host", w.ctypes.data, None if fs is None else fs.ctypes.data, cin, cout, kh, kw,
                  stride_w, pad_w, phase, dtype, out.ctypes.data)
        return out

# ... 44 lines not shown
```

### rangedet_amd/lower.py

```python
import os
from dataclasses import dataclass, field

from . import devswitch
from .lib import H16, RD_ADD, RD_BF16, RD_F16, RD_F32, RD_RELU_POST, RD_RELU_PRE


@dataclass
class TRef:
    buf: int
    C: int
    H: int
    W: int
    cs: int
    co: int = 0
    cmap: tuple = None
    tail: "TRef" = None


@dataclass
class FlatRef:
    buf: int
    shape: tuple


@dataclass
class Plan:
    dtype: int
    batch: int
    steps: list = field(default_factory=list)
    buffers: dict = field(default_factory=dict)
    outputs: list = field(default_factory=list)
    input_vars: dict = field(default_factory=dict)
    num_classes: int = 1


def conv_steps(steps):
    for st in steps:
        if st["kind"] in ("conv_pair", "block"):
            yield st["a"], 0.5
            yield st["b"], 0.5
        elif st["kind"] == "conv":
            yield st, 1
        elif st["kind"] == "deconv":
            yield st, 1 if st.get("one_launch") else st["stride_w"]


def _strip_cast(s):
    while s.op == "cast":
        s = s.inputs[0]
    return s


def _is(s, op, **attrs):
    return s.op == op and all(s.attrs.get(k) == v for k, v in attrs.items())


class Lowering:
    def __init__(self, group, input_shapes, dtype, batch):
        assert dtype in (RD_F32, RD_BF16, RD_F16)
        self.dtype = dtype
        self.h16 = dtype in H16
        self.esz = 2 if self.h16 else 4
        self.gran = 16 if self.h16 else 8
        self.B = batch
        self.shapes = dict(input_shapes)
        self.plan = Plan(dtype=dtype, batch=batch)
        self.memo = {}
        self.nbuf = 0
        self.consumers = {}
        self._count_consumers(group)
        for out in group.inputs:
            self.plan.outputs.append(self.emit_value(out))
        self._fuse_head_out()
        self._fuse_blocks()
        self._pair_equal_convs()
        self._mark_mfma16()

    def _mark_mfma16(self):
        if not self.h16 or devswitch.get("RD_NO_MFMA16"):
            return
        for st in self.plan.steps:
            if st["kind"] == "block" and st["a"]["cin"] == 64 and not devswitch.get("RD_NO_MFMA16_BLOCK"):
                st["m16"] = True
            if st["kind"] == "conv" and tuple(st["k"]) == (3, 3) and st["cout"] == 128 and st["stride_w"] == 1 and st.get("ex") and \
                    st.get("fold") and not st.get("sc") and st.get("x2") is None and not st.get("s2view"):
                cin = len(st["cmap"]) if st.get("cmap") else st["cin"]
                if cin % 32 == 0 and cin >= 32:
                    st["m16"] = True

    def _pair_equal_convs(self):
        if not self.h16 or devswitch.get("RD_PAIR", "0") in ("", "0"):
            return
        max_w = int(devswitch.get("RD_PAIR_MAXW", "100000"))
        same_input_only = devswitch.get("RD_PAIR", "0") == "2"

        def sig(st):
            if st["kind"] != "conv" or not st.get("ex") or not st.get("fold") or st.get("sc") or st.get("s2view") or st.get("x2") is not None:
                return None
            if st["res"] is not None or st["cout"] != 128 or st["stride_w"] != 1 or tuple(st["k"]) != (3, 3) or st["flags"] != RD_RELU_POST:
                return None
            x, o, h = st["x"], st["out"], st.get("head")
            if x.W > max_w:
                return None
            return (x.H, x.W, x.cs, len(st["cmap"]) if st.get("cmap") else st["cin"], o.cs if not h else None,
                    (h["n_off"], h["N"]) if h else None)

        def is_write(key):
            return key in ("out", "out1", "head_out", "head_out1", "keep") or key.startswith("out_")

        out, written, touched, open_ = [], {}, {}, {}
        for st in self.plan.steps:
            k = sig(st)
            if k is not None:
                ready = written.get(st["x"].buf, -1)
                clear = max((touched.get(v.buf, -1) for v in (st["out"], st.get("head_out")) if v is not None), default=-1)
                j = next((j for j in open_.get(k, []) if ready < j and clear < j and (not same_input_only or out[j]["x"] == st["x"])), None)
                if j is not None:
                    open_[k].remove(j)
                    a = out[j]
                    p = dict(kind="conv_pair", name=a["name"] + " + " + st["name"], a=a, b=st, x=a["x"], x1=st["x"], out=a["out"],
                             out1=st["out"])
                    if a.get("head"):
                        p["head_out"], p["head_out1"] = a["head_out"], st["head_out"]
                    out[j] = p
                    for v in (st["out"], st.get("head_out")):
                        if v is not None:
                            written[v.buf] = max(written.get(v.buf, -1), j)
                            touched[v.buf] = max(touched.get(v.buf, -1), j)
                    touched[st["x"].buf] = max(touched.get(st["x"].buf, -1), j)
                    continue
                open_.setdefault(k, []).append(len(out))
            def refs(key, v):
                if isinstance(v, (TRef, FlatRef)):
                    yield key, v
                    if isinstance(v, TRef) and v.tail is not None:
                        yield key, v.tail
                elif isinstance(v, dict):
                    for k2, v2 in v.items():
                        yield from refs(k2 if isinstance(k2, str) else key, v2)
                elif isinstance(v, (list, tuple)):
                    for v2 in v:
                        yield from refs(key, v2)
            for key, v in st.items():
                for k2, r in refs(key, v):
                    touched[r.buf] = len(out)
                    if is_write(k2):
                        written[r.buf] = len(out)
            out.append(st)
        self.plan.steps = out

    def _fuse_blocks(self):
        if not self.h16 or devswitch.get("RD_NO_FUSE_BLOCK"):
            return
        steps = self.plan.steps
        uses = {}

        def scan(i, key, v):
            if isinstance(v, (TRef, FlatRef)):
                uses.setdefault(v.buf, []).append((i, key))
                if isinstance(v, TRef) and v.tail is not None:
                    scan(i, key + ".tail", v.tail)
            elif isinstance(v, dict):
                for k2, v2 in v.items():
                    scan(i, key + "." + str(k2), v2)
            elif isinstance(v, (list, tuple)):
                for k2, v2 in enumerate(v):
                    scan(i, key + "." + str(k2), v2)
        for i, st in enumerate(steps):
            for key, v in st.items():
                scan(i, key, v)
        for o in (self.plan.outputs if isinstance(self.plan.outputs, (list, tuple)) else []):
            scan(-1, "output", o)

        def plain64(st, first=False):
            if not (st["kind"] == "conv" and tuple(st["k"]) == (3, 3) and st["stride_w"] == 1 and st["cout"] == 64 and st.get("ex") and
# ... 284 lines not shown
        for p, c, o in zip(parts, cs_list, offs):
            r = self.emit_act(p, dest=(out.buf, out.cs, o))
            if (r.H, r.W) != ref_hw:
                raise ValueError("concat %s: spatial mismatch" % s.name)
        return out

    def _match_meta(self, agg_conv):
        try:
            a = agg_conv.inputs[0]
            if not _is(a, "Activation", act_type="relu"):
                return None
            bn1 = a.inputs[0]
            if bn1.op != "BatchNorm" or bn1.inputs[0].op != "reshape":
                return None
            mul = bn1.inputs[0].inputs[0]
            if mul.op != "multiply":
                return None
        except (IndexError, AttributeError):
            return None
        ds, wts = mul.inputs
        if not (ds.op == "reshape" and ds.inputs[0].op == "im2col"):
            raise NotImplementedError("meta kernel: unexpected data-sample branch at %s" % mul.name)
        im_d = ds.inputs[0]
        data = im_d.inputs[0]
        if im_d.attrs != dict(kernel=(3, 3), stride=(1, 1), dilate=(1, 1), pad=(1, 1)):
            raise NotImplementedError("meta kernel: only 3x3/stride 1/pad 1 sampling")
        c1 = wts.inputs[0] if wts.op == "reshape" else None
        ok = c1 is not None and c1.op == "Convolution" and _is(c1.inputs[0], "Activation", act_type="relu")
        c0 = c1.inputs[0].inputs[0] if ok else None
        ok = ok and c0.op == "Convolution" and c0.inputs[0].op == "reshape" and c0.inputs[0].inputs[0].op == "broadcast_minus"
        if not ok:
            raise NotImplementedError("meta kernel: unexpected MLP branch (only fc+relu+fc without norm)")
        bm = c0.inputs[0].inputs[0]
        nb, ctr = bm.inputs
        if not (nb.op == "reshape" and nb.inputs[0].op == "im2col" and ctr.op == "expand_dims"):
            raise NotImplementedError("meta kernel: unexpected relative-coordinate branch")
        coord = _strip_cast(ctr.inputs[0])
        if _strip_cast(nb.inputs[0].inputs[0]).uid != coord.uid or coord.op != "var":
            raise NotImplementedError("meta kernel: coordinates must be one input variable")
        if (c0.attrs["num_filter"], c1.attrs["num_filter"], agg_conv.attrs["num_filter"]) != (32, 64, 64) or \
                c0.attrs["no_bias"] or c1.attrs["no_bias"] or not agg_conv.attrs["no_bias"]:
            raise NotImplementedError("meta kernel %s: MLP %d -> %d, aggregation to %d channels.  The fused Meta-Kernel is built for the shipped "
                                      "unit only: 3 -> 32 -> 64 MLP with biases (meta_kernel_units / fc channels of the reference config), "
                                      "64 data channels, 9 x 64 = 576 -> 64 aggregation without bias" %
                                      (agg_conv.name, c0.attrs["num_filter"], c1.attrs["num_filter"], agg_conv.attrs["num_filter"]))
        return dict(data=data, coord=coord.name, mlp0=c0.name, mlp1=c1.name, bn1=bn1.name, eps1=bn1.attrs["eps"])

    def _emit_meta(self, m, agg_conv, bn2, dest):
        x = self.emit_act(m["data"])
        if x.C != 64:
            raise NotImplementedError("meta kernel %s: %d data channels (the fused Meta-Kernel is built for 64)" % (agg_conv.name, x.C))
        cshape = self.want_input(m["coord"])
        if cshape != (3, x.H, x.W):
            raise ValueError("meta kernel: coord shape %s vs data %s" % (cshape, (x.H, x.W)))
        out = self._out(64, x.H, x.W, dest)
        self.step("meta", x=x, out=out, coord=m["coord"], mlp0=m["mlp0"], mlp1=m["mlp1"], bn1=m["bn1"], eps1=m["eps1"],
                  agg=agg_conv.name, bn2=bn2.name, eps2=bn2.attrs["eps"])
        return out

    def emit_value(self, s):
        s0 = s
        key = ("v", s.uid, s.index)
        if key in self.memo:
            return self.memo[key]
        if s.op == "var":
            self.plan.input_vars.setdefault(s.name, None)
            v = ("input", s.name)
        elif s.op == "zeros":
            v = ("zeros", s.attrs["shape"])
        elif s.op == "Custom" and s.attrs["op_type"] == "get_sorted_foreground":
            v = ("flat", self._sorted_fg(s)[s.index])
        elif s.op == "Custom" and s.attrs["op_type"] == "batch_rotated_iou":
            v = ("flat", self._batch_riou(s))
        elif s.op == "Decode3DBbox":
            v = ("flat", self._decode(s))
        elif s.op == "NMS3D":
            keep, final = self._nms3d(s)
            v = ("flat_i32", keep) if s.index == 0 else ("flat", final)
        else:
            raise NotImplementedError("graph output %r (op %s) has no HIP lowering" % (s0.name, s.op))
        self.memo[key] = v
        return v

    def _flat_levels(self, s, transposed):
        levels = s.inputs if s.op == "concat" else [s]
        out = []
        for lv in levels:
            q = lv
            if transposed:
                if not _is(q, "transpose", axes=(0, 2, 1)):
                    raise NotImplementedError("bbox_delta level is not transposed (0,2,1)")
                q = q.inputs[0]
            if q.op != "squeeze" or q.inputs[0].op != "slice_axis" or q.inputs[0].inputs[0].op != "reshape":
                raise NotImplementedError("per-class flatten chain not recognised at %s" % lv.name)
            sl = q.inputs[0]
            cls_i = sl.attrs["begin"]
            if sl.attrs["axis"] != 1 or sl.attrs["end"] != cls_i + 1:
                raise NotImplementedError("slice_axis %s" % sl.name)
            conv = _strip_cast(sl.inputs[0].inputs[0])
            if conv.op != "Convolution" or conv.attrs["kernel"] != (1, 1) or conv.attrs["no_bias"]:
                raise NotImplementedError("head output must be a 1x1 Convolution with bias at %s" % lv.name)
            out.append((conv, cls_i))
        return out

    def _sorted_fg(self, s):
        key = ("sfg", s.uid)
        if key in self.memo:
            return self.memo[key]
        score, delta, pc, mask = s.inputs
        apply_sigmoid = 0
        if _is(score, "Activation", act_type="sigmoid"):
            apply_sigmoid = 1
            score = score.inputs[0]
        lv_s = self._flat_levels(score, False)
        lv_d = self._flat_levels(delta, True)
        if len(lv_s) != len(lv_d):
            raise ValueError("score / delta level count")
        feats, N = [], 0
        for (cs_, ci), (cd_, di) in zip(lv_s, lv_d):
            fs = self.emit_act(cs_.inputs[0])
            fd = self.emit_act(cd_.inputs[0])
            feats.append((cs_, ci, fs, cd_, di, fd, N))
            N += fs.H * fs.W
        ncls = lv_s[0][0].attrs["num_filter"]
        D = lv_d[0][0].attrs["num_filter"] // ncls
        logit = FlatRef(self.new_buf(self.B * N * 4, persistent=True), (N,))
        dl = FlatRef(self.new_buf(self.B * N * D * 4, persistent=True), (N, D))
        for cs_, ci, fs, cd_, di, fd, off in feats:
            self.step("head_out", name=cs_.name, x=fs, out=logit, n_off=off, N=N, rows=(ci, ci + 1), nout=1)
            self.step("head_out", name=cd_.name, x=fd, out=dl, n_off=off, N=N, rows=(di * D, di * D + D), nout=D)
        pcs = self._concat_vars(pc, 3)
        msk = self._concat_vars(mask, None)
        k = int(s.attrs["num_fgs"])
        if N < k:
            raise ValueError("get_sorted_foreground: N (%d) < num_fgs (%d)" % (N, k))
        o_s = FlatRef(self.new_buf(self.B * k * 4, persistent=True), (k,))
        o_d = FlatRef(self.new_buf(self.B * k * D * 4), (k, D))
        o_p = FlatRef(self.new_buf(self.B * k * 3 * 4), (k, 3))
        self.step("sorted_fg", score=logit, delta=dl, pc=pcs, mask=msk, N=N, k=k, D=D, apply_sigmoid=apply_sigmoid,
                  out_score=o_s, out_delta=o_d, out_pc=o_p)
        self.memo[key] = (o_s, o_d, o_p)
        return self.memo[key]

    def _concat_vars(self, s, last):
        parts = s.inputs if s.op == "concat" else [s]
        names, n = [], 0
        for p in parts:
            p = _strip_cast(p)
            if p.op != "var":
                raise NotImplementedError("pc / mask inputs must be input variables")
            shp = self.want_input(p.name)
            names.append((p.name, shp[0]))
            n += shp[0]
        ref = FlatRef(self.new_buf(self.B * n * (last or 1) * 4, persistent=True), (n, last) if last else (n,))
        self.step("concat_in", names=names, out=ref, last=last or 1, N=n)
        return ref

    def _decode(self, s):
        d, p = s.inputs
        if not (d.op == "Custom" and p.op == "Custom" and d.uid == p.uid and d.index == 1 and p.index == 2):
            raise NotImplementedError("Decode3DBbox inputs must be outputs 1,2 of get_sorted_foreground")
        o_s, o_d, o_p = self._sorted_fg(d)
        k = o_d.shape[0]
        out = FlatRef(self.new_buf(self.B * k * 10 * 4, persistent=True), (k, 10))
        self.step("decode", delta=o_d, pc=o_p, out=out, k=k, box_type=o_d.shape[1], is_bin=int(s.attrs["is_bin"]))
        return out


    def _batch_riou(self, s):
        key = ("briou", s.uid)
        if key in self.memo:
            return self.memo[key]
        iou_type = s.attrs.get("iou_type", "bev")
        if iou_type not in ("bev", "3d"):
            raise ValueError("batch_rotated_iou: iou_type %r ('bev' or '3d')" % iou_type)
        gdim = 8 if iou_type == "bev" else 7
        prop, gt = s.inputs
        kind, boxes = self.emit_value(prop)
        gt = _strip_cast(gt)
        if kind != "flat" or len(boxes.shape) != 2 or boxes.shape[1] != 10 or gt.op != "var":
            raise NotImplementedError("batch_rotated_iou: proposal must be a (B,N,10) box tensor, gt_bbox an input variable")
        gshape = self.want_input(gt.name)
        if len(gshape) != 2 or gshape[1] != gdim or gshape[0] > 256:
            raise ValueError("batch_rotated_iou (%s): gt_bbox shape %s (need (n_gt <= 256, %d))" % (iou_type, gshape, gdim))
        out = FlatRef(self.new_buf(self.B * boxes.shape[0] * 4, persistent=True), (boxes.shape[0],))
        self.step("batch_riou", boxes=boxes, gt=gt.name, N=boxes.shape[0], n_gt=gshape[0], out=out, iou_type=iou_type)
        self.memo[key] = out
        return out

    def _nms3d(self, s):
        key = ("nms3d", s.uid)
        if key in self.memo:
            return self.memo[key]
        (bx,) = s.inputs
        if bx.op != "Decode3DBbox":
            raise NotImplementedError("NMS3D input must be the Decode3DBbox output (score-sorted boxes)")
        boxes = self._decode(bx)
        n, mk = boxes.shape[0], int(s.attrs["max_keep"])
        keep = FlatRef(self.new_buf(self.B * mk * 4, persistent=True), (mk,))
        final = FlatRef(self.new_buf(self.B * mk * 10 * 4, persistent=True), (mk, 10))
        self.step("nms3d", boxes=boxes, N=n, thr=float(s.attrs["iou_thres"]), max_keep=mk,
                  normal_iou=int(s.attrs["normal_iou"]), keep=keep, out=final)
        self.memo[key] = (keep, final)
        return self.memo[key]


def lower(test_symbol, input_shapes, dtype=RD_BF16, batch=1):
    return Lowering(test_symbol, input_shapes, dtype, batch).plan
```

### rangedet_amd/pipeline.py

```python
import os
import numpy as np

from . import devswitch, lib as rdlib
from .config import rangedet_veh_wo_aug_4_18e as cfgmod
from .lower import lower
from .runtime import Executor, TorchAllocator


def input_shapes(H, W, strides=(1, 2, 4), channels=8):
    shapes = {'input_data': (channels, H, W), 'coord_s1': (3, H, W)}
    for s in strides:
        shapes['pc_vehicle_frame_s%d' % s] = (H * W // s, 3)
        shapes['range_image_mask_s%d' % s] = (H * W // s,)
    return shapes



def _stream_prio(var):
    return int(devswitch.get(var, "0"))


class BatchPostProcessor:

    def __init__(self, B, k, min_score, thr_lo, thr_hi, is_3d_iou, lib, alloc, cap=4096, hash_scale=100, tie_order="reference", wnms_diag=0):
        self.B, self.k, self.cap = B, k, min(cap, k, rdlib.RD_WNMS_MAX_K)
        self.hash_scale, self.tie_order = int(hash_scale), tie_order
        self.wnms_diag = int(wnms_diag)
        self.min_score, self.thr_lo, self.thr_hi, self.is3d = min_score, thr_lo, thr_hi, int(is_3d_iou)
        self.L, self.A = lib, alloc
        A, L = alloc, lib
        self.dets = A.alloc(B * k * 12 * 4)
        self.count = A.alloc(max(16, 4 * B), zero=True)
        self.ws_f_bytes = L.raw("rd_score_filter_workspace_bytes")(k) * B
        self.ws_f = A.alloc(self.ws_f_bytes)
        self.ws_w_bytes = L.raw("rd_wnms_workspace_bytes")(self.cap) * B
        self.ws_w = A.alloc(self.ws_w_bytes)
        self.out = A.alloc(B * self.cap * 12 * 4)
        self.keep = A.alloc(B * self.cap * 4)
        self.nkeep = A.alloc(max(16, 4 * B), zero=True)
        self.out8 = A.alloc(B * self.cap * 8 * 4)
        self.identity = A.upload(np.arange(self.cap, dtype=np.int32))
        self._host = None

    def enqueue_filter(self, score_ptr, score_bs, box_ptr, box_bs, stream=None):
        L, A = self.L, self.A
        st = A.stream_ptr(stream) if hasattr(A, "stream_ptr") else A.stream
        L.call("rd_score_filter_dets_batched", score_ptr, score_bs, box_ptr, box_bs, self.k, self.min_score, A.ptr(self.dets),
               self.k * 12, A.ptr(self.count), A.ptr(self.ws_f), self.ws_f_bytes, self.B, st)

    def enqueue_nms(self, stream=None):
        L, A = self.L, self.A
        st = A.stream_ptr(stream) if hasattr(A, "stream_ptr") else A.stream
        order = A.ptr(self.identity) if self.tie_order == "stable" else None
        L.call("rd_wnms_4c_batched", A.ptr(self.dets), self.k * 12, self.cap, A.ptr(self.count), order, 0,
               rdlib.RD_TIE_REFERENCE | self.wnms_diag, self.thr_lo, self.thr_hi, self.is3d, self.hash_scale, A.ptr(self.out), self.cap * 12,
               A.ptr(self.keep), self.cap, A.ptr(self.nkeep), A.ptr(self.ws_w), self.ws_w_bytes, self.B, st)
        L.call("rd_dets12_to_8_batched", A.ptr(self.out), self.cap * 12, self.cap, A.ptr(self.nkeep), A.ptr(self.out8),
               self.cap * 8, self.B, st)

    def collect_all(self, done=None):
        A = self.A
        if done is not None and hasattr(done, "synchronize"):
            done.synchronize()
        else:
            A.sync()
        count = np.array(A.to_numpy(A.view_i32(self.count, (self.B,))))
        nkeep = np.array(A.to_numpy(A.view_i32(self.nkeep, (self.B,))))
        if int(count.max()) > self.cap:
            raise rdlib.RangeDetError(rdlib.RD_EWORKSPACE, "%d detections above min_score exceed the WNMS capacity %d" % (int(count.max()), self.cap))
        m = int(nkeep.max()) if self.B else 0
        rows = np.array(A.to_numpy(A.view_f32(self.out, (self.B, self.cap, 12))[:, :m]))
        keep = np.array(A.to_numpy(A.view_i32(self.keep, (self.B, self.cap))[:, :m]))
        d8 = np.array(A.to_numpy(A.view_f32(self.out8, (self.B, self.cap, 8))[:, :m]))
        return [dict(num_candidates=int(count[b]), wnms_rows=rows[b, :nkeep[b]].copy(), keep_inds=keep[b, :nkeep[b]].copy(),
                     det_xyzlwhyaws=d8[b, :nkeep[b]].copy()) for b in range(self.B)]

    def collect(self, b=0):
        return self.collect_all()[b]


class Nms3dPostProcessor:

    def __init__(self, B, k, max_keep, min_score, lib, alloc):
        self.B, self.k, self.mk, self.min_score, self.L, self.A = B, k, max_keep, min_score, lib, alloc
        A, L = alloc, lib
        self.cap = max_keep
        self.kscore = A.alloc(B * max_keep * 4)
        self.dets = A.alloc(B * max_keep * 12 * 4)
        self.count = A.alloc(max(16, 4 * B), zero=True)
        self.ws_bytes = L.raw("rd_score_filter_workspace_bytes")(max_keep) * B
        self.ws = A.alloc(self.ws_bytes)
        self.out8 = A.alloc(B * max_keep * 8 * 4)
        self._keep = None

    def enqueue(self, score_ptr, score_bs, final_ptr, keep_ptr, keep_view, stream=None):
        L, A, mk = self.L, self.A, self.mk
        st = A.stream_ptr(stream) if hasattr(A, "stream_ptr") else A.stream
        self._keep = keep_view
        L.call("rd_gather_keep_scores", score_ptr, score_bs, self.k, keep_ptr, mk, A.ptr(self.kscore), self.B, st)
        L.call("rd_score_filter_dets_batched", A.ptr(self.kscore), mk, final_ptr, mk * 10, mk, self.min_score, A.ptr(self.dets),
               mk * 12, A.ptr(self.count), A.ptr(self.ws), self.ws_bytes, self.B, st)
        L.call("rd_dets12_to_8_batched", A.ptr(self.dets), mk * 12, mk, A.ptr(self.count), A.ptr(self.out8), mk * 8, self.B, st)

    def collect_all(self, done=None):
        if done is not None and hasattr(done, "synchronize"):
            done.synchronize()
        else:
            self.A.sync()
        return [self._collect(b) for b in range(self.B)]

    def collect(self, b=0):
        self.A.sync()
        return self._collect(b)

    def _collect(self, b):
        A = self.A
        K = int(A.to_numpy(A.view_i32(self.count, (self.B,)))[b])
        rows = A.to_numpy(A.view_f32(self.dets, (self.B, self.mk, 12)))[b, :K].copy()
        d8 = A.to_numpy(A.view_f32(self.out8, (self.B, self.mk, 8)))[b, :K].copy()
        keep = np.array(A.to_numpy(self._keep))[b]
        sc = A.to_numpy(A.view_f32(self.kscore, (self.B, self.mk)))[b]
        keep = keep[(keep >= 0) & (sc > self.min_score)]
        return dict(num_candidates=K, wnms_rows=rows, keep_inds=keep, det_xyzlwhyaws=d8)


class _FrameView:

    def __init__(self, bp, b):
        self.bp, self.b = bp, b
        self.cap = bp.cap

    def collect(self):
        return self.bp.collect(self.b)

    def out_rows(self):
        A = self.bp.A
        return A.view_f32(self.bp.out, (self.bp.B, self.bp.cap, 12))[self.b]

    def nkeep_view(self):
        A = self.bp.A
        return A.view_i32(self.bp.nkeep, (self.bp.B,))[self.b:self.b + 1]


class RangeDetPipeline:
    def __init__(self, params, dtype=rdlib.RD_BF16, feat_size=(64, 2650), pad_field=(64, 2656), batch=1,
                 pre_nms_top_n=50000, wnms_cap=4096, variant="veh", lib=None, alloc=None, wnms=True, tie_order="reference",
                 hash_scale=100, wnms_diag=0, graph=False):
        topn = pre_nms_top_n if isinstance(pre_nms_top_n, dict) else {cfgmod.variant_classes(variant)[0]: pre_nms_top_n}
        self.cfg = cfgmod.get_config(False, variant=variant, feat_size=feat_size, pad_field=pad_field,
                                     batch_image=batch, pre_nms_top_n=topn, wnms=wnms)
        self.wnms = bool(wnms)
        General, RpnParam, ModelParam, TestParam = self.cfg[0], self.cfg[2], self.cfg[6], self.cfg[8]
        self.lib = lib or rdlib.get_lib()
        self.alloc = alloc or TorchAllocator()
        self.class_names = tuple(General.class_names)
        nch = cfgmod.KITTI_INPUT_CHANNELS if variant == "kitti" else 8
        self.plan = lower(ModelParam.test_symbol, input_shapes(*pad_field, channels=nch), dtype, batch)
        self.exe = Executor(self.plan, params, self.lib, self.alloc)
        self.ks = {c: RpnParam.all_proposal.rpn_pre_nms_top_n[c] for c in self.class_names}
        self.batch = batch
        self.use_graph = bool(graph) and hasattr(self.alloc, "torch")
        self._graphs = {}
        self._capture_stream = None
        self.max_graphs = 8
        self.graph_replays = 0
        self._post_stream = None
        self.post_on_launch_stream = not devswitch.get("RD_POST_SIDE_STREAM")
        self._filter_done = None
        self._post_done = None
        assert self.wnms or len(self.class_names) == 1, "the NMS3D branch is single-class (tools/test.py:182)"
        self.bposts = {}
        for c in self.class_names:
            if self.wnms:
                self.bposts[c] = BatchPostProcessor(batch, self.ks[c], TestParam.min_score[c], TestParam.nms.thr_lo,
                                                    TestParam.nms.thr_hi, TestParam.nms.is_3d_iou, self.lib, self.alloc, wnms_cap,
                                                    hash_scale=hash_scale, tie_order=tie_order, wnms_diag=wnms_diag)
            else:
                self.bposts[c] = Nms3dPostProcessor(batch, self.ks[c], RpnParam.all_proposal.rpn_post_nms_top_n[c],
                                                    TestParam.min_score[c], self.lib, self.alloc)
        self.k = self.ks[self.class_names[0]]
        self.bpost = self.bposts[self.class_names[0]]
        self.post = [_FrameView(self.bpost, b) for b in range(batch)]

    def forward(self, inputs):
        return self.exe.forward(inputs)

    def enqueue(self, inputs):
        if self.use_graph:
            outs = self._enqueue_graph(inputs)
            if outs is not None:
                return outs
        return self._enqueue_eager(inputs)

    def _record(self, inputs):
        outs = self.exe.forward(inputs)
        ptr = lambda t: self.alloc.ptr(t) if hasattr(t, "data_ptr") else t.ctypes.data
        if not self.wnms:
            self.bpost.enqueue(ptr(outs[1]), self.k, ptr(outs[2]), ptr(outs[3]), outs[3], stream=None)
            return outs
# ... 117 lines not shown
```

### rangedet_amd/runtime.py

```python
import os

import numpy as np

from . import devswitch, lib as rdlib
from .lower import FlatRef, TRef


class TorchAllocator:

    def __init__(self, device="cuda:0", stream=None):
        import torch
        if not torch.cuda.is_available():
            raise RuntimeError("rangedet_amd needs a ROCm GPU (torch.cuda.is_available() is False); there is no CPU fallback")
        self.torch = torch
        self.device = torch.device(device)
        torch.cuda.set_device(self.device)
        self._stream = stream

    @property
    def stream(self):
        st = self._stream or self.torch.cuda.current_stream(self.device)
        return st.cuda_stream

    def alloc(self, nbytes, zero=False):
        f = self.torch.zeros if zero else self.torch.empty
        return f(max(int(nbytes), 16), dtype=self.torch.uint8, device=self.device)

    def upload(self, arr):
        a = np.ascontiguousarray(arr)
        t = self.torch.from_numpy(a.view(np.uint8).reshape(-1)).to(self.device)
        return t

    def ptr(self, buf):
        return buf.data_ptr()

    def view_f32(self, buf, shape):
        n = int(np.prod(shape))
        return buf[: n * 4].view(self.torch.float32).view(*shape)

    def view_i32(self, buf, shape):
        n = int(np.prod(shape))
        return buf[: n * 4].view(self.torch.int32).view(*shape)

    def to_numpy(self, t):
        return t.detach().cpu().numpy()

    def as_device_f32(self, x):
        t = self.torch
        if isinstance(x, np.ndarray):
            return t.from_numpy(np.ascontiguousarray(x, dtype=np.float32)).to(self.device)
        return x.to(device=self.device, dtype=t.float32).contiguous()

    def assign(self, dst_view, src):
        dst_view.copy_(src.reshape(dst_view.shape))

    def new_stream(self, priority=0):
        return self.torch.cuda.Stream(device=self.device, priority=priority)

    def stream_ptr(self, stream):
        return stream.cuda_stream if stream is not None else self.stream

    def record_event(self, stream=None):
        ev = self.torch.cuda.Event()
        ev.record(stream if stream is not None else self.torch.cuda.current_stream(self.device))
        return ev

    def wait_event(self, ev, stream=None):
        (stream if stream is not None else self.torch.cuda.current_stream(self.device)).wait_event(ev)

    def sync(self):
        self.torch.cuda.synchronize(self.device)


def bn_affine(P, name, eps, pad_to=None):
    g, b, m, v = (np.asarray(P[name + s], np.float64) for s in ("_gamma", "_beta", "_moving_mean", "_moving_var"))
    s = g / np.sqrt(v + eps)
    s, t = s.astype(np.float32), (b - m * s).astype(np.float32)
    if pad_to is not None and pad_to > len(s):
        s = np.concatenate([s, np.ones(pad_to - len(s), np.float32)])
        t = np.concatenate([t, np.zeros(pad_to - len(t), np.float32)])
    return s, t


def pad_rows(w, n, axis=0):
    if w.shape[axis] >= n:
        return w
    shp = list(w.shape)
    shp[axis] = n - w.shape[axis]
    return np.concatenate([w, np.zeros(shp, w.dtype)], axis)


class Executor:
    def __init__(self, plan, params, lib=None, alloc=None, reuse_buffers=True, keep_sorted_idx=False):
        self.keep_sorted_idx = keep_sorted_idx
        self.plan = plan
        self.lib = lib or rdlib.get_lib()
        self.alloc = alloc or TorchAllocator()
        self.dtype = plan.dtype
        self.B = plan.batch
        self._phys = {}
        self._assign_buffers(reuse_buffers)
        self._bound = [self._bind(st, params) for st in plan.steps]

    def _assign_buffers(self, reuse):
        plan = self.plan
        last_use, first_def = {}, {}
        for i, st in enumerate(plan.steps):
            for v in st.values():
                if isinstance(v, (TRef, FlatRef)):
                    last_use[v.buf] = i
                    first_def.setdefault(v.buf, i)
        for kind, v in plan.outputs:
            if kind in ("flat", "flat_i32"):
                last_use[v.buf] = len(plan.steps) + 1
        free = {}
        release = {}
        for b, i in last_use.items():
            release.setdefault(i, []).append(b)
        order = sorted(plan.buffers, key=lambda b: first_def.get(b, 0))
        by_def = {}
        for b in order:
            by_def.setdefault(first_def.get(b, 0), []).append(b)
        for i in range(len(plan.steps) + 2):
            for b in by_def.get(i, []):
                info = plan.buffers[b]
                if reuse and not info["persistent"] and free.get(info["nbytes"]):
                    self._phys[b] = free[info["nbytes"]].pop()
                else:
                    self._phys[b] = self.alloc.alloc(info["nbytes"], zero=info["zero"])
            for b in release.get(i, []):
                info = plan.buffers[b]
                if reuse and not info["persistent"] and last_use[b] <= len(plan.steps):
                    free.setdefault(info["nbytes"], []).append(self._phys[b])
        self.device_bytes = sum(int(t.numel()) if hasattr(t, "numel") else len(t) for t in {id(v): v for v in self._phys.values()}.values())

    def p(self, ref):
        return self.alloc.ptr(self._phys[ref.buf])

    def _bind(self, st, P):
        L, A, dt = self.lib, self.alloc, self.dtype
        k = st["kind"]
        b = dict(st)
        if k == "conv_pair":
            b["a"], b["b"] = self._bind(st["a"], P), self._bind(st["b"], P)
            return b
        if k == "block":
            ca, cb = st["a"], st["b"]
            w1, w2 = (np.asarray(P[c["name"] + "_weight"], np.float32) for c in (ca, cb))
            if ca.get("cmap"):
                wp = np.zeros((w1.shape[0], len(ca["cmap"])) + w1.shape[2:], np.float32)
                for pc, lc in enumerate(ca["cmap"]):
                    if lc >= 0:
                        wp[:, pc] = w1[:, lc]
                w1 = wp
            (s1, t1), (s2, t2) = bn_affine(P, ca["bn"], ca["eps"]), bn_affine(P, cb["bn"], cb["eps"])
            m16 = bool(st.get("m16")) and w1.shape[1] == 64
            b["m16"] = m16
            b["w"] = A.upload(L.pack_block64(w1, s1, w2, s2, dtype=dt, m16=m16))
            b["shift1"] = A.upload(t1)
            b["sc_w"] = None
            if cb.get("sc"):
                sc = cb["sc"]
                wsc = np.asarray(P[sc["name"] + "_weight"], np.float32).reshape(64, -1)
                if sc.get("cmap"):
                    wq = np.zeros((64, len(sc["cmap"])), np.float32)
                    for pc, lc in enumerate(sc["cmap"]):
                        if lc >= 0:
                            wq[:, pc] = wsc[:, lc]
                    wsc = wq
                ss, ts = bn_affine(P, sc["bn"], sc["eps"])
                b["sc_w"] = A.upload(L.pack_conv1x1_sc_m16(wsc, ss, dtype=dt) if m16 else L.pack_conv1x1_sc(wsc, fold_scale=ss, dtype=dt))
                t2 = (t2.astype(np.float64) + ts).astype(np.float32)
            b["shift2"] = A.upload(t2)
            b["cin"] = w1.shape[1]
            return b
        if k == "conv":
            w = pad_rows(np.asarray(P[st["name"] + "_weight"], np.float32), st["cout"])
            if st.get("cmap"):
                wp = np.zeros((w.shape[0], len(st["cmap"])) + w.shape[2:], np.float32)
                for pc, lc in enumerate(st["cmap"]):
                    if lc >= 0:
                        wp[:, pc] = w[:, lc]
                w = wp
            s, t = bn_affine(P, st["bn"], st["eps"], pad_to=st["cout"])
            if st.get("sc"):
                sc = st["sc"]
                wsc = np.asarray(P[sc["name"] + "_weight"], np.float32)
                wsc = pad_rows(wsc.reshape(wsc.shape[0], -1), st["cout"])
                if sc.get("cmap"):
                    wq = np.zeros((w.shape[0], len(sc["cmap"])), np.float32)
                    for pc, lc in enumerate(sc["cmap"]):
                        if lc >= 0:
                            wq[:, pc] = wsc[:, lc]
                    wsc = wq
                ss, ts = bn_affine(P, sc["bn"], sc["eps"], pad_to=st["cout"])
                b["w"] = A.upload(L.pack_conv3x3_ex(w, st["stride_w"], st["x"].cs, fold_scale=s, dtype=dt))
                b["sc_w"] = A.upload(L.pack_conv1x1_sc(wsc, fold_scale=ss, dtype=dt))
                b["scale"], b["shift"] = None, A.upload((t.astype(np.float64) + ts).astype(np.float32))
            elif st.get("x2") is not None:
                b["w"] = A.upload(L.pack_conv3x3_cat(w, st["x"].C, st["x2"].cs, fold_scale=s, dtype=dt))
                b["scale"], b["shift"] = None, A.upload(t)
                b["flags"] = st["flags"] | rdlib.RD_SCALE_FOLDED
            elif st.get("ex") and st.get("fold") and st.get("m16") and \
                    L.raw("rd_conv3x3_mfma16_ok")(w.shape[1], st["cout"], 1, st["x"].W, 1 if st.get("head") else 0) == 1:
                b["w"] = A.upload(L.pack_conv3x3_m16(w, s, dtype=dt))
                b["scale"], b["shift"] = None, A.upload(t)
                b["flags"] = st["flags"] | rdlib.RD_SCALE_FOLDED | rdlib.RD_MFMA16
            elif st.get("ex") and st.get("fold"):
                b["w"] = A.upload(L.pack_conv3x3_ex(w, st["stride_w"], st["x"].cs, fold_scale=s, dtype=dt))
                b["scale"], b["shift"] = None, A.upload(t)
                b["flags"] = st["flags"] | rdlib.RD_SCALE_FOLDED
            elif st.get("ex"):
                b["w"] = A.upload(L.pack_conv3x3_ex(w, st["stride_w"], st["x"].cs, dtype=dt))
                b["scale"], b["shift"] = A.upload(s), A.upload(t)
            else:
                b["w"] = A.upload(L.pack_conv_weight(w, dt))
                b["scale"], b["shift"] = A.upload(s), A.upload(t)
        elif k == "deconv":
            w = pad_rows(np.asarray(P[st["name"] + "_weight"], np.float32), st["cout"], axis=1)
            s, t = bn_affine(P, st["bn"], st["eps"], pad_to=st["cout"])
            fs = s if st.get("fold") else None
            imgs = [L.pack_deconv_weight(w, st["stride_w"], st["pad_w"], ph, dt, fold_scale=fs) for ph in range(st["stride_w"])]
            b["all_phases"] = bool(st.get("one_launch")) and len({len(i) for i in imgs}) == 1 and \
                L.raw("rd_deconv2d_all_phases_ok")(st["k"][0], st["k"][1], st["stride_w"], st["pad_w"], st["cout"], dt) == 1
            if st.get("one_launch") and not b["all_phases"] and not L.raw("rd_deconv2d_all_phases_ok")(st["k"][0], st["k"][1], st["stride_w"], st["pad_w"], st["cout"], dt):
                b["one_launch"] = False
            if b["all_phases"]:
                b["w_all"], b["w_pb"] = A.upload(np.concatenate(imgs)), len(imgs[0])
            r_, o_ = st["res"], st["out"]
            b["pairs"] = b["all_phases"] and not devswitch.get("RD_DECONV_NO_PAIRS") and o_.cs == st["cout"] and o_.co == 0 and \
                (r_ is None or (r_.cs == st["cout"] and r_.co == 0)) and \
                L.raw("rd_deconv2d_phase_pairs_ok")(st["k"][0], st["k"][1], st["stride_w"], st["pad_w"], st["cout"], dt) == 1
            if b["pairs"]:
                pimgs = [L.pack_deconv_phase_pair(imgs[p], imgs[p + 1], st["cin"], dt) for p in range(0, st["stride_w"], 2)]
                b["w_pairs"], b["w_pairb"], b["shift2"] = A.upload(np.concatenate(pimgs)), len(pimgs[0]), A.upload(np.concatenate([t, t]))
            b["w"] = [A.upload(i) for i in imgs]
            b["scale"], b["shift"] = (None if st.get("fold") else A.upload(s)), A.upload(t)
            if st.get("fold"):
                b["flags"] = st["flags"] | rdlib.RD_SCALE_FOLDED
        elif k == "meta":
            s1, t1 = bn_affine(P, st["bn1"], st["eps1"])
            s2, t2 = bn_affine(P, st["bn2"], st["eps2"])
            pk = L.pack_meta(P[st["mlp0"] + "_weight"].reshape(32, 3), P[st["mlp0"] + "_bias"],
                             P[st["mlp1"] + "_weight"].reshape(64, 32), P[st["mlp1"] + "_bias"], s1, t1,
                             P[st["agg"] + "_weight"].reshape(64, 576), s2, t2, dt)
            b["packed"] = A.upload(pk)
        if k == "conv" and st.get("head"):
            h = st["head"]
            r0, r1 = h["rows"]
            hw = np.asarray(P[h["name"] + "_weight"], np.float32).reshape(-1, st["cout"])[r0:r1]
            b["head_w"] = A.upload(L.pack_head_weight(hw, dtype=dt, m16=bool(b.get("flags", 0) & rdlib.RD_MFMA16)))
            b["head_bias"] = A.upload(np.asarray(P[h["name"] + "_bias"], np.float32)[r0:r1])
        elif k == "head_out":
            r0, r1 = st["rows"]
            w = np.asarray(P[st["name"] + "_weight"], np.float32).reshape(-1, st["x"].C)[r0:r1]
            b["w"] = A.upload(w)
            b["bias"] = A.upload(np.asarray(P[st["name"] + "_bias"], np.float32)[r0:r1])
        elif k == "nms3d":
            nb = L.raw("rd_nms3d_workspace_bytes")(st["N"], self.B)
            b["ws"] = A.alloc(nb)
            b["ws_bytes"] = nb
        elif k == "sorted_fg":
            nb = L.raw("rd_sorted_foreground_workspace_bytes")(st["N"], st["k"]) * self.B
            b["ws"] = A.alloc(nb)
            b["ws_bytes"] = nb
            b["idx"] = A.alloc(self.B * st["k"] * 4) if self.keep_sorted_idx else None
        return b

    def forward(self, inputs, only=None, dev=None):
        L, A, dt, B = self.lib, self.alloc, self.dtype, self.B
        st_ = A.stream
        dev = {} if dev is None else dev

        def din(name):
            if name not in dev:
                dev[name] = A.as_device_f32(inputs[name])
            return dev[name]

        steps = self._bound if only is None else [self._bound[only]]
        for b in steps:
            k = b["kind"]
            if k == "nchw_in":
                o = b["out"]
                src = din(b["name"])
                assert tuple(src.shape) == (B, o.C, o.H, o.W), (b["name"], tuple(src.shape), (B, o.C, o.H, o.W))
                L.call("rd_nchw_to_nhwc", A.ptr(src), self.p(o), B, o.C, o.H, o.W, o.cs, o.co, b["zero_pad"], dt, st_)
            elif k == "block":
                x, o = b["x"], b["out"]
                if b.get("m16"):
                    L.call("rd_block64_m16_bn_act", self.p(x), x.cs, x.co, A.ptr(b["w"]), A.ptr(b["shift1"]), A.ptr(b["shift2"]),
                           A.ptr(b["sc_w"]) if b["sc_w"] is not None else None, self.p(o), o.cs, o.co, B, x.H, x.W, dt, st_)
                else:
                    L.call("rd_block64_bn_act", self.p(x), x.cs, x.co, b["cin"], A.ptr(b["w"]), A.ptr(b["shift1"]), A.ptr(b["shift2"]),
                           A.ptr(b["sc_w"]) if b["sc_w"] is not None else None, self.p(o), o.cs, o.co, B, x.H, x.W, dt, st_)
            elif k == "conv_pair":
                p, q = b["a"], b["b"]
                x0, x1 = p["x"], q["x"]
                cin = len(p["cmap"]) if p.get("cmap") else p["cin"]
                if p.get("head"):
                    h0, h1 = p["head"], q["head"]
                    L.call("rd_conv2d_bn_act_head_out_pair",
                           self.p(x0), x0.co, A.ptr(p["w"]), A.ptr(p["shift"]), A.ptr(p["head_w"]), A.ptr(p["head_bias"]),
                           self.p(h0["out"]), h0["N"] * h0["nout"], h0["nout"],
                           self.p(x1), x1.co, A.ptr(q["w"]), A.ptr(q["shift"]), A.ptr(q["head_w"]), A.ptr(q["head_bias"]),
                           self.p(h1["out"]), h1["N"] * h1["nout"], h1["nout"],
                           x0.cs, h0["n_off"], B, x0.H, x0.W, cin, p["flags"], dt, st_)
                else:
                    o0, o1 = p["out"], q["out"]
                    L.call("rd_conv3x3_bn_act_pair", self.p(x0), x0.co, A.ptr(p["w"]), A.ptr(p["shift"]), self.p(o0), o0.co,
                           self.p(x1), x1.co, A.ptr(q["w"]), A.ptr(q["shift"]), self.p(o1), o1.co, x0.cs, o0.cs, B, x0.H, x0.W, cin,
                           p["flags"], dt, st_)
            elif k == "conv" and b.get("head"):
                x, h = b["x"], b["head"]
                L.call("rd_conv2d_bn_act_head_out", self.p(x), x.cs, x.co, A.ptr(b["w"]),
                       A.ptr(b["scale"]) if b["scale"] is not None else None, A.ptr(b["shift"]), B,
                       x.H, x.W, b["cin"], b["flags"], A.ptr(b["head_w"]), A.ptr(b["head_bias"]), self.p(h["out"]),
                       h["N"] * h["nout"], h["n_off"], h["nout"], dt, st_)
            elif k == "conv" and b.get("x2") is not None:
                x, x2, o = b["x"], b["x2"], b["out"]
                L.call("rd_conv3x3_bn_act_cat", self.p(x), x.cs, x.co, x.C, self.p(x2), x2.cs, x2.co, x2.cs, A.ptr(b["w"]), A.ptr(b["shift"]),
                       self.p(o), o.cs, o.co, B, x.H, x.W, b["cout"], b["flags"], dt, st_)
            elif k == "conv" and b.get("ex"):
                x, o, r, sx = b["x"], b["out"], b["res"], b.get("sc_x")
                cin = len(b["cmap"]) if b.get("cmap") else b["cin"]
                L.call("rd_conv3x3_bn_act_ex", self.p(x), x.cs, x.co, A.ptr(b["w"]), A.ptr(b["scale"]) if b["scale"] is not None else None,
                       A.ptr(b["shift"]), self.p(r) if r else None, r.cs if r else 0, r.co if r else 0,
                       self.p(sx) if sx else None, sx.cs if sx else 0, sx.co if sx else 0,
                       (len(b["sc"]["cmap"]) if b["sc"].get("cmap") else b["sc"]["cin"]) if sx else 0,
                       A.ptr(b["sc_w"]) if sx else None, self.p(o), o.cs, o.co, B, x.H, x.W, cin, b["cout"], b["stride_w"],
                       b["flags"], dt, st_)
            elif k == "conv":
                x, o, r = b["x"], b["out"], b["res"]
                L.call("rd_conv2d_bn_act", self.p(x), x.cs, x.co, A.ptr(b["w"]), A.ptr(b["scale"]), A.ptr(b["shift"]),
                       self.p(r) if r else None, r.cs if r else 0, r.co if r else 0, self.p(o), o.cs, o.co, B, x.H, x.W,
                       b["cin"], b["cout"], b["k"][0], b["k"][1], b["stride_w"], b["flags"], dt, st_)
            elif k == "deconv":
                x, o, r = b["x"], b["out"], b["res"]
                if b.get("pairs"):
                    L.call("rd_deconv2d_bn_act_pairs", self.p(x), x.cs, x.co, A.ptr(b["w_pairs"]), b["w_pairb"], A.ptr(b["shift2"]), self.p(r), r.cs,
                           r.co, self.p(o), o.cs, o.co, B, x.H, x.W, b["cin"], b["cout"], b["k"][0], b["k"][1], b["stride_w"], b["pad_w"],
                           b["flags"], dt, st_)
                    continue
                if b.get("all_phases"):
                    L.call("rd_deconv2d_bn_act_all", self.p(x), x.cs, x.co, A.ptr(b["w_all"]), b["w_pb"], A.ptr(b["shift"]), self.p(r), r.cs,
                           r.co, self.p(o), o.cs, o.co, B, x.H, x.W, b["cin"], b["cout"], b["k"][0], b["k"][1], b["stride_w"], b["pad_w"],
                           b["flags"], dt, st_)
                    continue
                for ph in range(b["stride_w"]):
                    L.call("rd_deconv2d_bn_act", self.p(x), x.cs, x.co, A.ptr(b["w"][ph]),
                           A.ptr(b["scale"]) if b["scale"] is not None else None, A.ptr(b["shift"]), self.p(r), r.cs, r.co, self.p(o), o.cs, o.co, B, x.H, x.W, b["cin"],
                           b["cout"], b["k"][0], b["k"][1], b["stride_w"], b["pad_w"], ph, b["flags"], dt, st_)
            elif k == "meta":
                x, o = b["x"], b["out"]
                c = din(b["coord"])
                assert tuple(c.shape) == (B, 3, x.H, x.W)
                L.call("rd_meta_kernel_fwd", self.p(x), x.cs, x.co, A.ptr(c), A.ptr(b["packed"]), self.p(o), o.cs, o.co,
                       B, x.H, x.W, dt, st_)
            elif k == "head_out":
                x, o = b["x"], b["out"]
                L.call("rd_head_out", self.p(x), x.cs, x.co, A.ptr(b["w"]), A.ptr(b["bias"]), self.p(o),
                       b["N"] * b["nout"], b["n_off"], B, x.H, x.W, x.C, b["nout"], dt, st_)
            elif k == "concat_in":
                o = b["out"]
                row = b["N"] * b["last"] * 4
                off = 0
                for name, n in b["names"]:
                    src = din(name)
                    assert tuple(src.shape)[:2] == (B, n), (name, tuple(src.shape))
                    L.call("rd_copy_rows", A.ptr(src), n * b["last"] * 4, self.p(o), row, off * b["last"] * 4,
                           n * b["last"] * 4, B, st_)
                    off += n
            elif k == "sorted_fg":
                L.call("rd_sorted_foreground", self.p(b["score"]), self.p(b["delta"]), self.p(b["pc"]), self.p(b["mask"]),
                       B, b["N"], b["k"], b["D"], b["apply_sigmoid"], self.p(b["out_score"]), self.p(b["out_delta"]),
                       self.p(b["out_pc"]), A.ptr(b["idx"]) if b["idx"] is not None else None, A.ptr(b["ws"]), b["ws_bytes"], st_)
            elif k == "decode":
                L.call("rd_decode3d_bbox", self.p(b["delta"]), self.p(b["pc"]), self.p(b["out"]), B, b["k"],
                       b["box_type"], b["is_bin"], st_)
            elif k == "batch_riou":
                g = din(b["gt"])
                three_d = b.get("iou_type", "bev") == "3d"
                assert tuple(g.shape) == (B, b["n_gt"], 7 if three_d else 8), (b["gt"], tuple(g.shape))
                L.call("rd_batch_rotated_iou_3d" if three_d else "rd_batch_rotated_iou", self.p(b["boxes"]), 10, A.ptr(g), self.p(b["out"]),
                       None, B, b["N"], b["n_gt"], st_)
            elif k == "nms3d":
                L.call("rd_nms3d", self.p(b["boxes"]), B, b["N"], b["thr"], b["max_keep"], b["normal_iou"], self.p(b["keep"]),
                       self.p(b["out"]), A.ptr(b["ws"]), b["ws_bytes"], st_)
            else:
                raise RuntimeError("unknown plan step %r" % k)
        if only is not None:
            return None
        outs = []
        for kind, v in self.plan.outputs:
            if kind == "flat":
                outs.append(A.view_f32(self._phys[v.buf], (B,) + tuple(v.shape)))
            elif kind == "flat_i32":
                outs.append(A.view_i32(self._phys[v.buf], (B,) + tuple(v.shape)))
            elif kind == "input":
                outs.append(inputs.get(v))
            else:
                outs.append(np.zeros(v, np.float32))
        return outs

    def read_flat(self, ref):
        self.alloc.sync()
        return np.array(self.alloc.to_numpy(self.alloc.view_f32(self._phys[ref.buf], (self.B,) + tuple(ref.shape))))

    def sorted_idx(self, which=0):
        b = [x for x in self._bound if x["kind"] == "sorted_fg"][which]
        self.alloc.sync()
        return np.array(self.alloc.to_numpy(self.alloc.view_i32(b["idx"], (self.B, b["k"]))))

    def debug_tensor(self, ref):
        A, L = self.alloc, self.lib
        out = A.alloc(self.B * ref.C * ref.H * ref.W * 4)
        L.call("rd_nhwc_to_nchw", self.p(ref), A.ptr(out), self.B, ref.C, ref.H, ref.W, ref.cs, ref.co, self.dtype, A.stream)
        A.sync()
        return A.to_numpy(A.view_f32(out, (self.B, ref.C, ref.H, ref.W)))
```

Baseline: 1018.

## Fuse post-processing: segmented inputs, keygen+histogram, decode in gather, sorted filter

Post-processing now reads point-cloud and mask inputs directly from their per-part buffers instead of first concatenating them with copy kernels. Key generation is merged with the top-k histogram pass, and 3D box decoding is folded into the sorted gather kernel. Because the input is already sorted, the score filter becomes a single kernel that drops the count/scan/scatter passes. This removes several launches and intermediate HBM round trips, at the cost of extra index arithmetic and a sorted-input assumption in the filter.

```diff
diff --git a/include/rangedet_hip.h b/include/rangedet_hip.h
--- a/include/rangedet_hip.h
+++ b/include/rangedet_hip.h
@@ -130,6 +130,12 @@
                          int B, long N, long k, int D, int apply_sigmoid, float* out_score, float* out_delta,
                          float* out_pc, int* out_idx, void* ws, size_t ws_bytes, void* stream);
 
+int rd_sorted_foreground_decode(const float* cls_score, const float* bbox_delta, const float* const* pc_parts,
+                                const long* pc_part_n, int n_pc_parts, const float* const* mask_parts,
+                                const long* mask_part_n, int n_mask_parts, int B, long N, long k, int D, int apply_sigmoid,
+                                int is_bin, float* out_score, float* out_delta, float* out_pc, int* out_idx,
+                                float* out_box, void* ws, size_t ws_bytes, void* stream);
+
 int rd_decode3d_bbox(const float* bbox_delta, const float* pc, float* out, int B, long N, int box_type,
                      int is_bin, void* stream);
 
@@ -139,6 +145,9 @@
 int rd_score_filter_dets_batched(const float* scores, long scores_bstride, const float* boxes10, long boxes_bstride,
                                  long n, float min_score, float* dets, long dets_bstride, int* d_count, void* ws,
                                  size_t ws_bytes, int B, void* stream);
+int rd_score_filter_dets_sorted_batched(const float* scores, long scores_bstride, const float* boxes10,
+                                        long boxes_bstride, long n, float min_score, float* dets, long dets_bstride,
+                                        int* d_count, int B, void* stream);
 
 #define RD_WNMS_MAX_K 65536
 #define RD_TIE_STABLE 0
diff --git a/rangedet_amd/csrc/k_misc.h b/rangedet_amd/csrc/k_misc.h
--- a/rangedet_amd/csrc/k_misc.h
+++ b/rangedet_amd/csrc/k_misc.h
@@ -175,12 +175,8 @@
   }
 }
 
-__global__ __launch_bounds__(256) void decode3d_kernel(const float* __restrict__ delta, const float* __restrict__ pc,
-                                                       float* __restrict__ out, long n, int box_type, int is_bin) {
-  long idx = blockIdx.x * 256L + threadIdx.x;
-  if (idx >= n) return;
-  const float* d = delta + idx * box_type;
-  float pc_x = pc[idx * 3 + 0], pc_y = pc[idx * 3 + 1], pc_z = pc[idx * 3 + 2];
+__device__ __forceinline__ void decode3d_box(const float* d, float pc_x, float pc_y, float pc_z, int is_bin, float* __restrict__ o) {
+  _Pragma("clang fp contract(off)")
   float az = atan2f(pc_y, pc_x);
   float ca = cosf(az), sa = sinf(az);
   float dx, dy, width, length, height, z0, yaw_l;
@@ -202,21 +198,28 @@
     z0 = d[6];
     yaw_l = atan2f(d[5], d[4]) + az;
   }
-  float dxl = dx * ca - dy * sa;
-  float dyl = dx * sa + dy * ca;
+  float dxl = fmaf(dx, ca, -(dy * sa));
+  float dyl = fmaf(dy, ca, dx * sa);
   float cx = pc_x + dxl, cy = pc_y + dyl;
   float sy = sinf(yaw_l), cyw = cosf(yaw_l);
   float hl = (float)(0.5 * (double)length), hw = (float)(0.5 * (double)width);
-  float hx[4] = {hl, -hl, -hl, hl};
-  float hy[4] = {-hw, -hw, hw, hw};
-  float* o = out + idx * 10;
-#pragma unroll
-  for (int k = 0; k < 4; ++k) {
-    o[2 * k] = (hx[k] * cyw - hy[k] * sy) + cx;
-    o[2 * k + 1] = (hx[k] * sy + hy[k] * cyw) + cy;
-  }
+  const float shw = sy * hw, shl = sy * hl, chw = cyw * hw;
+  o[0] = fmaf(cyw, hl, shw) + cx;
+  o[1] = fmaf(sy, hl, -chw) + cy;
+  o[2] = fmaf(cyw, -hl, shw) + cx;
+  o[3] = fmaf(cyw, -hw, -shl) + cy;
+  o[4] = fmaf(cyw, -hl, -shw) + cx;
+  o[5] = fmaf(sy, -hl, chw) + cy;
+  o[6] = fmaf(cyw, hl, -shw) + cx;
+  o[7] = fmaf(sy, hl, chw) + cy;
   o[8] = z0;
   o[9] = z0 + height;
+}
+__global__ __launch_bounds__(256) void decode3d_kernel(const float* __restrict__ delta, const float* __restrict__ pc,
+                                                       float* __restrict__ out, long n, int box_type, int is_bin) {
+  long idx = blockIdx.x * 256L + threadIdx.x;
+  if (idx >= n) return;
+  decode3d_box(delta + idx * box_type, pc[idx * 3 + 0], pc[idx * 3 + 1], pc[idx * 3 + 2], is_bin, out + idx * 10);
 }
 
 __global__ __launch_bounds__(256) void filter_count_kernel(const float* __restrict__ scores, long n, float thr,
@@ -287,6 +290,29 @@
     d[11] = scores[i];
   }
 }
+__global__ __launch_bounds__(256) void filter_sorted_kernel(const float* __restrict__ scores, const float* __restrict__ boxes10,
+                                                            long n, float thr, float* __restrict__ dets, int* __restrict__ d_count,
+                                                            long sc_bs, long box_bs, long dets_bs) {
+  scores += blockIdx.y * sc_bs;
+  boxes10 += blockIdx.y * box_bs;
+  dets += blockIdx.y * dets_bs;
+  const long i = blockIdx.x * 256L + threadIdx.x;
+  if (i >= n) return;
+  const float s = scores[i];
+  if (!(s > thr)) {
+    if (i == 0) d_count[blockIdx.y] = 0;
+    return;
+  }
+  if (i + 1 == n || !(scores[i + 1] > thr)) d_count[blockIdx.y] = (int)(i + 1);
+  const float* b = boxes10 + i * 10;
+  float* d = dets + (size_t)i * 12;
+#pragma unroll
+  for (int k = 0; k < 8; ++k) d[k] = b[k];
+  d[8] = fdlibm_atan2f(b[1] - b[3], b[0] - b[2]);
+  d[9] = b[8];
+  d[10] = b[9] - b[8];
+  d[11] = s;
+}
 
 __global__ __launch_bounds__(256) void dets12_to_8_kernel(const float* __restrict__ d12, int cap, const int* __restrict__ d_count,
                                                           float* __restrict__ o8, long d12_bs, long o8_bs) {
diff --git a/rangedet_amd/csrc/k_sort.h b/rangedet_amd/csrc/k_sort.h
--- a/rangedet_amd/csrc/k_sort.h
+++ b/rangedet_amd/csrc/k_sort.h
@@ -16,16 +16,36 @@
   return __uint_as_float(u);
 }
 
-__global__ __launch_bounds__(256) void sort_keygen_kernel(const float* __restrict__ score, const float* __restrict__ mask,
-                                                          long N, int apply_sigmoid, unsigned* __restrict__ keys,
+struct FlatSegs {
+  const float* p[4];
+  long n[4];
+  long bs[4];
+  int nseg;
+};
+__device__ __forceinline__ const float* flat_seg_row(const FlatSegs& s, long b, long i, int last) {
+  const float* p = s.p[0];
+  long bs = s.bs[0], off = 0;
+  const long e0 = s.n[0], e1 = e0 + s.n[1], e2 = e1 + s.n[2];
+  if (s.nseg > 1 && i >= e0) { p = s.p[1]; bs = s.bs[1]; off = e0; }
+  if (s.nseg > 2 && i >= e1) { p = s.p[2]; bs = s.bs[2]; off = e1; }
+  if (s.nseg > 3 && i >= e2) { p = s.p[3]; bs = s.bs[3]; off = e2; }
+  return p + b * bs + (i - off) * last;
+}
+
+__device__ __forceinline__ unsigned sort_score_key(const float* __restrict__ score, const FlatSegs& mask, long b, long bm, long N,
+                                                   long i, int apply_sigmoid) {
+  float s = score[b * N + i];
+  if (apply_sigmoid) s = 1.0f / (1.0f + expf(-s));
+  if (mask.nseg) s = s * *flat_seg_row(mask, bm, i, 1);
+  return desc_key(s);
+}
+__global__ __launch_bounds__(256) void sort_keygen_kernel(const float* __restrict__ score, const FlatSegs mask, long b0, long N,
+                                                          int apply_sigmoid, unsigned* __restrict__ keys,
                                                           unsigned* __restrict__ idx, long ws_stride) {
   long i = blockIdx.x * 256L + threadIdx.x;
   if (i >= N) return;
   const long b = blockIdx.y;
-  float s = score[b * N + i];
-  if (apply_sigmoid) s = 1.0f / (1.0f + expf(-s));
-  if (mask) s = s * mask[b * N + i];
-  keys[b * ws_stride + i] = desc_key(s);
+  keys[b * ws_stride + i] = sort_score_key(score, mask, b, b0 + b, N, i, apply_sigmoid);
   idx[b * ws_stride + i] = (unsigned)i;
 }
 __global__ __launch_bounds__(256) void sort_keygen_dets_kernel(const float* __restrict__ dets, int cap,
@@ -138,26 +158,39 @@
   }
 }
 
+template <bool DEC>
 __global__ __launch_bounds__(256) void sort_gather_kernel(const unsigned* __restrict__ keys, const unsigned* __restrict__ idx,
-                                                          long k, int D, const float* __restrict__ delta,
-                                                          const float* __restrict__ pc, float* __restrict__ out_score,
-                                                          float* __restrict__ out_delta, float* __restrict__ out_pc,
-                                                          int* __restrict__ out_idx, long ws_stride, long N) {
+                                                          long k, int D, const float* __restrict__ delta, const FlatSegs pc, long b0,
+                                                          float* __restrict__ out_score, float* __restrict__ out_delta,
+                                                          float* __restrict__ out_pc, int* __restrict__ out_idx,
+                                                          float* __restrict__ out_box, int is_bin, long ws_stride, long N) {
   long i = blockIdx.x * 256L + threadIdx.x;
   if (i >= k) return;
-  {
-    const long b = blockIdx.y;
+  const long b = blockIdx.y;
+  {
     keys += b * ws_stride; idx += b * ws_stride;
-    delta += b * N * D; pc += b * N * 3;
+    delta += b * N * D;
     out_score += b * k; out_delta += b * k * D; out_pc += b * k * 3;
     if (out_idx) out_idx += b * k;
   }
   unsigned j = idx[i];
   out_score[i] = key_to_float(keys[i]);
-  for (int c = 0; c < D; ++c) out_delta[i * D + c] = delta[(size_t)j * D + c];
-  out_pc[i * 3 + 0] = pc[(size_t)j * 3 + 0];
-  out_pc[i * 3 + 1] = pc[(size_t)j * 3 + 1];
-  out_pc[i * 3 + 2] = pc[(size_t)j * 3 + 2];
+  const float* p = flat_seg_row(pc, b0 + b, (long)j, 3);
+  const float px = p[0], py = p[1], pz = p[2];
+  if (DEC) {
+    float d[8];
+#pragma unroll
+    for (int c = 0; c < 8; ++c) d[c] = c < D ? delta[(size_t)j * D + c] : 0.f;
+#pragma unroll
+    for (int c = 0; c < 8; ++c)
+      if (c < D) out_delta[i * D + c] = d[c];
+    decode3d_box(d, px, py, pz, is_bin, out_box + (b * k + i) * 10);
+  } else {
+    for (int c = 0; c < D; ++c) out_delta[i * D + c] = delta[(size_t)j * D + c];
+  }
+  out_pc[i * 3 + 0] = px;
+  out_pc[i * 3 + 1] = py;
+  out_pc[i * 3 + 2] = pz;
   if (out_idx) out_idx[i] = (int)j;
 }
 
@@ -177,6 +210,27 @@
   for (int i = threadIdx.x; i < SEL_BINS; i += 256)
     if (h[i]) atomicAdd(&h12[i], h[i]);
 }
+__global__ __launch_bounds__(256) void sort_keygen_hist_kernel(const float* __restrict__ score, const FlatSegs mask, long b0, long N,
+                                                               int apply_sigmoid, unsigned* __restrict__ keys,
+                                                               unsigned* __restrict__ h12, long ws_stride) {
+  const long b = blockIdx.y;
+  keys += b * ws_stride; h12 += b * ws_stride;
+  __shared__ unsigned h[SEL_BINS];
+  for (int i = threadIdx.x; i < SEL_BINS; i += 256) h[i] = 0;
+  __syncthreads();
+  const long base = (long)blockIdx.x * SORT_TILE;
+  for (int r = 0; r < SORT_TILE / 256; ++r) {
+    const long i = base + r * 256 + threadIdx.x;
+    if (i < N) {
+      const unsigned key = sort_score_key(score, mask, b, b0 + b, N, i, apply_sigmoid);
+      keys[i] = key;
+      atomicAdd(&h[key >> SEL_SHIFT], 1u);
+    }
+  }
+  __syncthreads();
+  for (int i = threadIdx.x; i < SEL_BINS; i += 256)
+    if (h[i]) atomicAdd(&h12[i], h[i]);
+}
 __global__ __launch_bounds__(256) void select_thresh_kernel(const unsigned* __restrict__ h12, long k, unsigned* __restrict__ sel,
                                                             long ws_stride) {
   h12 += blockIdx.y * ws_stride; sel += blockIdx.y * ws_stride;
@@ -226,7 +280,8 @@
                                                              unsigned* __restrict__ idx_out, long ws_stride) {
   {
     const long o = blockIdx.y * ws_stride;
-    keys_in += o; idx_in += o; sel += o; cnt += o; keys_out += o; idx_out += o;
+    keys_in += o; sel += o; cnt += o; keys_out += o; idx_out += o;
+    if (idx_in) idx_in += o;
   }
   const unsigned T = sel[0];
   __shared__ unsigned wcnt[4][8], sbase;
@@ -244,7 +299,7 @@
     const long i = base + r * 64 + lane;
     const bool valid = i < N;
     key[r] = valid ? keys_in[i] : 0xFFFFFFFFu;
-    id[r] = valid ? idx_in[i] : 0u;
+    id[r] = !valid ? 0u : idx_in ? idx_in[i] : (unsigned)i;
     m[r] = __ballot(valid && (key[r] >> SEL_SHIFT) <= T);
     if (lane == 0) wcnt[wv][r] = (unsigned)__popcll(m[r]);
   }
@@ -307,17 +362,24 @@
   return check_launch("radix_sort_pairs");
 }
 
-inline int radix_topk_pairs(const SortWs& s, long N, long k, hipStream_t st, int nb, long ws_stride, unsigned** rk, unsigned** ri) {
-  const bool off = dev_switches().sort_no_select;
+inline bool topk_preselects(long N, long k) { return !dev_switches().sort_no_select && 2 * k <= N; }
+inline int radix_topk_pairs(const SortWs& s, long N, long k, hipStream_t st, int nb, long ws_stride, unsigned** rk, unsigned** ri,
+                            bool keyed = false) {
   *rk = s.keysA; *ri = s.idxA;
   RD_REQUIRE(k > 0 && k <= N, RD_ESHAPE, "top-k: k %ld of N %ld", k, N);
-  if (off || 2 * k > N) return radix_sort_pairs(s, N, st, nb, ws_stride);
-  { int rc = sort_clear(s, st, nb, ws_stride, true); if (rc != RD_OK) return rc; }
-  hipLaunchKernelGGL(select_hist_kernel, dim3(s.nblk, nb), dim3(256), 0, st, s.keysA, N, s.h12, ws_stride);
+  if (!topk_preselects(N, k)) {
+    RD_REQUIRE(!keyed, RD_EINVAL, "top-k: keys without indices on the full-sort path");
+    return radix_sort_pairs(s, N, st, nb, ws_stride);
+  }
+  if (!keyed) {
+    int rc = sort_clear(s, st, nb, ws_stride, true);
+    if (rc != RD_OK) return rc;
+    hipLaunchKernelGGL(select_hist_kernel, dim3(s.nblk, nb), dim3(256), 0, st, s.keysA, N, s.h12, ws_stride);
+  }
   hipLaunchKernelGGL(select_thresh_kernel, dim3(1, nb), dim3(256), 0, st, s.h12, k, s.sel, ws_stride);
   hipLaunchKernelGGL(select_count_kernel, dim3(s.nblk, nb), dim3(256), 0, st, s.keysA, N, s.sel, s.cnt, ws_stride);
-  hipLaunchKernelGGL(select_compact_kernel, dim3(s.nblk, nb), dim3(256), 0, st, s.keysA, s.idxA, N, s.sel, s.cnt, s.keysB, s.idxB,
-                     ws_stride);
+  hipLaunchKernelGGL(select_compact_kernel, dim3(s.nblk, nb), dim3(256), 0, st, s.keysA, keyed ? nullptr : s.idxA, N, s.sel, s.cnt,
+                     s.keysB, s.idxB, ws_stride);
   SortWs v = s;
   v.keysA = s.keysB; v.keysB = s.keysA; v.idxA = s.idxB; v.idxB = s.idxA;
   *rk = s.keysB; *ri = s.idxB;
diff --git a/rangedet_amd/csrc/rd_api.hip b/rangedet_amd/csrc/rd_api.hip
--- a/rangedet_amd/csrc/rd_api.hip
+++ b/rangedet_amd/csrc/rd_api.hip
@@ -654,16 +654,28 @@
 }
 
 size_t rd_sorted_foreground_workspace_bytes(long N, long k) { (void)k; return (sort_ws_bytes(N) + 256 + 255) & ~(size_t)255; }
-int rd_sorted_foreground(const float* cls_score, const float* bbox_delta, const float* pc, const float* mask, int B,
-                         long N, long k, int D, int apply_sigmoid, float* out_score, float* out_delta, float* out_pc,
-                         int* out_idx, void* ws, size_t ws_bytes, void* stream) {
-  RD_REQUIRE(cls_score && bbox_delta && pc && out_score && out_delta && out_pc && ws, RD_EINVAL, "sorted_foreground: null pointer");
+static int make_segs(FlatSegs& s, const float* const* parts, const long* part_n, int nparts, int last, long N, const char* what) {
+  memset(&s, 0, sizeof(s));
+  RD_REQUIRE(nparts >= 1 && nparts <= 4 && parts && part_n, RD_ESHAPE, "sorted_foreground: %s in %d parts (1 to 4)", what, nparts);
+  long sum = 0;
+  for (int l = 0; l < nparts; ++l) {
+    RD_REQUIRE(parts[l] && part_n[l] > 0, RD_EINVAL, "sorted_foreground: %s part %d is empty", what, l);
+    s.p[l] = parts[l]; s.n[l] = part_n[l]; s.bs[l] = part_n[l] * last;
+    sum += part_n[l];
+  }
+  RD_REQUIRE(sum == N, RD_ESHAPE, "sorted_foreground: %s parts hold %ld rows, N is %ld", what, sum, N);
+  s.nseg = nparts;
+  return RD_OK;
+}
+static int sorted_foreground_impl(const float* cls_score, const float* bbox_delta, const FlatSegs& pcs, const FlatSegs& msk, int B,
+                                  long N, long k, int D, int apply_sigmoid, float* out_score, float* out_delta, float* out_pc,
+                                  int* out_idx, float* out_box, int is_bin, void* ws, size_t ws_bytes, hipStream_t st) {
+  RD_REQUIRE(cls_score && bbox_delta && out_score && out_delta && out_pc && ws, RD_EINVAL, "sorted_foreground: null pointer");
   RD_REQUIRE(B > 0 && N > 0 && k > 0 && D > 0, RD_ESHAPE, "sorted_foreground: empty shape");
   RD_REQUIRE(N >= k, RD_ESHAPE, "sorted_foreground: N (%ld) < num_fgs (%ld)", N, k);
   RD_REQUIRE(N < (1L << 31), RD_ESHAPE, "sorted_foreground: N too large");
   RD_REQUIRE(ws_bytes >= rd_sorted_foreground_workspace_bytes(N, k), RD_EWORKSPACE, "sorted_foreground: workspace %zu < %zu",
              ws_bytes, rd_sorted_foreground_workspace_bytes(N, k));
-  hipStream_t st = (hipStream_t)stream;
   void* wsa = (void*)(((uintptr_t)ws + 255) & ~(uintptr_t)255);
   SortWs s = sort_ws_carve(wsa, N);
   ProfScope ps(RD_PROF_SORT, st);
@@ -671,18 +683,62 @@
   const bool wide = ws_bytes >= per * (size_t)B;
   const long stride = wide ? (long)(per / 4) : 0;
   const int nb = wide ? B : 1;
+  const bool sel = topk_preselects(N, k);
   for (int b0 = 0; b0 < B; b0 += nb) {
-    hipLaunchKernelGGL(sort_keygen_kernel, dim3((unsigned)((N + 255) / 256), nb), dim3(256), 0, st, cls_score + (size_t)b0 * N,
-                       mask ? mask + (size_t)b0 * N : nullptr, N, apply_sigmoid, s.keysA, s.idxA, stride);
+    if (sel) {
+      int rc = sort_clear(s, st, nb, stride, true);
+      if (rc != RD_OK) return rc;
+      hipLaunchKernelGGL(sort_keygen_hist_kernel, dim3(s.nblk, nb), dim3(256), 0, st, cls_score + (size_t)b0 * N, msk, (long)b0, N,
+                         apply_sigmoid, s.keysA, s.h12, stride);
+    } else {
+      hipLaunchKernelGGL(sort_keygen_kernel, dim3((unsigned)((N + 255) / 256), nb), dim3(256), 0, st, cls_score + (size_t)b0 * N, msk,
+                         (long)b0, N, apply_sigmoid, s.keysA, s.idxA, stride);
+    }
     unsigned *rk, *ri;
-    int rc = radix_topk_pairs(s, N, k, st, nb, stride, &rk, &ri);
+    int rc = radix_topk_pairs(s, N, k, st, nb, stride, &rk, &ri, sel);
     if (rc != RD_OK) return rc;
-    hipLaunchKernelGGL(sort_gather_kernel, dim3((unsigned)((k + 255) / 256), nb), dim3(256), 0, st, rk, ri, k, D,
-                       bbox_delta + (size_t)b0 * N * D, pc + (size_t)b0 * N * 3, out_score + (size_t)b0 * k,
-                       out_delta + (size_t)b0 * k * D, out_pc + (size_t)b0 * k * 3, out_idx ? out_idx + (size_t)b0 * k : nullptr,
-                       stride, N);
+    const dim3 grid((unsigned)((k + 255) / 256), nb);
+    float* os = out_score + (size_t)b0 * k;
+    float* od = out_delta + (size_t)b0 * k * D;
+    float* op = out_pc + (size_t)b0 * k * 3;
+    int* oi = out_idx ? out_idx + (size_t)b0 * k : nullptr;
+    if (out_box)
+      hipLaunchKernelGGL(sort_gather_kernel<true>, grid, dim3(256), 0, st, rk, ri, k, D, bbox_delta + (size_t)b0 * N * D, pcs, (long)b0,
+                         os, od, op, oi, out_box + (size_t)b0 * k * 10, is_bin, stride, N);
+    else
+      hipLaunchKernelGGL(sort_gather_kernel<false>, grid, dim3(256), 0, st, rk, ri, k, D, bbox_delta + (size_t)b0 * N * D, pcs, (long)b0,
+                         os, od, op, oi, (float*)nullptr, 0, stride, N);
   }
   return check_launch("sorted_foreground");
+}
+
+int rd_sorted_foreground(const float* cls_score, const float* bbox_delta, const float* pc, const float* mask, int B,
+                         long N, long k, int D, int apply_sigmoid, float* out_score, float* out_delta, float* out_pc,
+                         int* out_idx, void* ws, size_t ws_bytes, void* stream) {
+  RD_REQUIRE(pc, RD_EINVAL, "sorted_foreground: null pointer");
+  RD_REQUIRE(N > 0, RD_ESHAPE, "sorted_foreground: empty shape");
+  FlatSegs pcs, msk;
+  int rc = make_segs(pcs, &pc, &N, 1, 3, N, "pc");
+  if (rc != RD_OK) return rc;
+  memset(&msk, 0, sizeof(msk));
+  if (mask && (rc = make_segs(msk, &mask, &N, 1, 1, N, "mask")) != RD_OK) return rc;
+  return sorted_foreground_impl(cls_score, bbox_delta, pcs, msk, B, N, k, D, apply_sigmoid, out_score, out_delta, out_pc, out_idx,
+                                nullptr, 0, ws, ws_bytes, (hipStream_t)stream);
+}
+
+int rd_sorted_foreground_decode(const float* cls_score, const float* bbox_delta, const float* const* pc_parts, const long* pc_part_n,
+                                int n_pc_parts, const float* const* mask_parts, const long* mask_part_n, int n_mask_parts, int B,
+                                long N, long k, int D, int apply_sigmoid, int is_bin, float* out_score, float* out_delta,
+                                float* out_pc, int* out_idx, float* out_box, void* ws, size_t ws_bytes, void* stream) {
+  RD_REQUIRE(!out_box || (is_bin && D == 7) || (!is_bin && D == 8), RD_ESHAPE,
+             "sorted_foreground_decode: box_type %d with is_bin=%d (8 for regular, 7 for bin)", D, is_bin);
+  FlatSegs pcs, msk;
+  int rc = make_segs(pcs, pc_parts, pc_part_n, n_pc_parts, 3, N, "pc");
+  if (rc != RD_OK) return rc;
+  memset(&msk, 0, sizeof(msk));
+  if (n_mask_parts > 0 && (rc = make_segs(msk, mask_parts, mask_part_n, n_mask_parts, 1, N, "mask")) != RD_OK) return rc;
+  return sorted_foreground_impl(cls_score, bbox_delta, pcs, msk, B, N, k, D, apply_sigmoid, out_score, out_delta, out_pc, out_idx,
+                                out_box, is_bin, ws, ws_bytes, (hipStream_t)stream);
 }
 
 int rd_decode3d_bbox(const float* bbox_delta, const float* pc, float* out, int B, long N, int box_type, int is_bin,
@@ -716,6 +772,16 @@
   hipLaunchKernelGGL(filter_scatter_kernel, dim3(nblk, B), dim3(256), 0, st, scores, boxes10, n, min_score, blk, dets,
                      scores_bstride, boxes_bstride, blk_bs, dets_bstride);
   return check_launch("score_filter");
+}
+int rd_score_filter_dets_sorted_batched(const float* scores, long scores_bstride, const float* boxes10, long boxes_bstride, long n,
+                                        float min_score, float* dets, long dets_bstride, int* d_count, int B, void* stream) {
+  RD_REQUIRE(scores && boxes10 && dets && d_count, RD_EINVAL, "score_filter_sorted: null pointer");
+  RD_REQUIRE(n > 0 && B > 0, RD_ESHAPE, "score_filter_sorted: empty input");
+  hipStream_t st = (hipStream_t)stream;
+  ProfScope ps(RD_PROF_WNMS, st);
+  hipLaunchKernelGGL(filter_sorted_kernel, dim3((unsigned)((n + 255) / 256), B), dim3(256), 0, st, scores, boxes10, n, min_score, dets,
+                     d_count, scores_bstride, boxes_bstride, dets_bstride);
+  return check_launch("score_filter_sorted");
 }
 int rd_score_filter_dets(const float* scores, const float* boxes10, long n, float min_score, float* dets, int* d_count,
                          void* ws, size_t ws_bytes, void* stream) {
diff --git a/rangedet_amd/lib.py b/rangedet_amd/lib.py
--- a/rangedet_amd/lib.py
+++ b/rangedet_amd/lib.py
@@ -91,11 +91,16 @@
     "rd_sorted_foreground_workspace_bytes": (c_size_t, [c_long, c_long]),
     "rd_sorted_foreground": (c_int, [c_void_p, c_void_p, c_void_p, c_void_p, c_int, c_long, c_long, c_int, c_int,
                                      c_void_p, c_void_p, c_void_p, c_void_p, c_void_p, c_size_t, c_void_p]),
+    "rd_sorted_foreground_decode": (c_int, [c_void_p, c_void_p, c_void_p, c_void_p, c_int, c_void_p, c_void_p, c_int, c_int, c_long,
+                                            c_long, c_int, c_int, c_int, c_void_p, c_void_p, c_void_p, c_void_p, c_void_p, c_void_p,
+                                            c_size_t, c_void_p]),
     "rd_decode3d_bbox": (c_int, [c_void_p, c_void_p, c_void_p, c_int, c_long, c_int, c_int, c_void_p]),
     "rd_score_filter_workspace_bytes": (c_size_t, [c_long]),
     "rd_score_filter_dets": (c_int, [c_void_p, c_void_p, c_long, c_float, c_void_p, c_void_p, c_void_p, c_size_t, c_void_p]),
     "rd_score_filter_dets_batched": (c_int, [c_void_p, c_long, c_void_p, c_long, c_long, c_float, c_void_p, c_long, c_void_p,
                                              c_void_p, c_size_t, c_int, c_void_p]),
+    "rd_score_filter_dets_sorted_batched": (c_int, [c_void_p, c_long, c_void_p, c_long, c_long, c_float, c_void_p, c_long, c_void_p,
+                                                    c_int, c_void_p]),
     "rd_wnms_workspace_bytes": (c_size_t, [c_int]),
     "rd_wnms_4c_batched": (c_int, [c_void_p, c_long, c_int, c_void_p, c_void_p, c_long, c_int, c_float, c_float, c_int, c_int,
                                    c_void_p, c_long, c_void_p, c_long, c_void_p, c_void_p, c_size_t, c_int, c_void_p]),
diff --git a/rangedet_amd/lower.py b/rangedet_amd/lower.py
--- a/rangedet_amd/lower.py
+++ b/rangedet_amd/lower.py
@@ -21,6 +21,13 @@
 class FlatRef:
     buf: int
     shape: tuple
+
+
+@dataclass
+class InputParts:
+    names: tuple
+    last: int
+    N: int
 
 
 @dataclass
@@ -611,6 +618,8 @@
             shp = self.want_input(p.name)
             names.append((p.name, shp[0]))
             n += shp[0]
+        if not devswitch.get("RD_NO_POST_FUSE"):
+            return InputParts(tuple(names), last or 1, n)
         ref = FlatRef(self.new_buf(self.B * n * (last or 1) * 4, persistent=True), (n, last) if last else (n,))
         self.step("concat_in", names=names, out=ref, last=last or 1, N=n)
         return ref
diff --git a/rangedet_amd/pipeline.py b/rangedet_amd/pipeline.py
--- a/rangedet_amd/pipeline.py
+++ b/rangedet_amd/pipeline.py
@@ -41,10 +41,15 @@
         self.out8 = A.alloc(B * self.cap * 8 * 4)
         self.identity = A.upload(np.arange(self.cap, dtype=np.int32))
         self._host = None
+        self.sorted_filter = not devswitch.get("RD_NO_POST_FUSE")
 
     def enqueue_filter(self, score_ptr, score_bs, box_ptr, box_bs, stream=None):
         L, A = self.L, self.A
         st = A.stream_ptr(stream) if hasattr(A, "stream_ptr") else A.stream
+        if self.sorted_filter:
+            L.call("rd_score_filter_dets_sorted_batched", score_ptr, score_bs, box_ptr, box_bs, self.k, self.min_score,
+                   A.ptr(self.dets), self.k * 12, A.ptr(self.count), self.B, st)
+            return
         L.call("rd_score_filter_dets_batched", score_ptr, score_bs, box_ptr, box_bs, self.k, self.min_score, A.ptr(self.dets),
                self.k * 12, A.ptr(self.count), A.ptr(self.ws_f), self.ws_f_bytes, self.B, st)
 
diff --git a/rangedet_amd/runtime.py b/rangedet_amd/runtime.py
--- a/rangedet_amd/runtime.py
+++ b/rangedet_amd/runtime.py
@@ -1,9 +1,10 @@
+import ctypes
 import os
 
 import numpy as np
 
 from . import devswitch, lib as rdlib
-from .lower import FlatRef, TRef
+from .lower import FlatRef, InputParts, TRef
 
 
 class TorchAllocator:
@@ -101,6 +102,7 @@
         self._phys = {}
         self._assign_buffers(reuse_buffers)
         self._bound = [self._bind(st, params) for st in plan.steps]
+        self._fuse_decode()
 
     def _assign_buffers(self, reuse):
         plan = self.plan
@@ -136,6 +138,28 @@
 
     def p(self, ref):
         return self.alloc.ptr(self._phys[ref.buf])
+
+    def _fuse_decode(self):
+        if devswitch.get("RD_NO_POST_FUSE"):
+            return
+        sfgs = {}
+        for b in self._bound:
+            if b["kind"] == "sorted_fg":
+                sfgs[(b["out_delta"].buf, b["out_pc"].buf)] = b
+            elif b["kind"] == "decode":
+                s = sfgs.get((b["delta"].buf, b["pc"].buf))
+                if s is not None and "decode" not in s and b["box_type"] == s["D"]:
+                    s["decode"], b["fused"] = b, True
+
+    def _parts(self, ref, din):
+        B = self.B
+        srcs = []
+        for name, n in ref.names:
+            src = din(name)
+            assert tuple(src.shape) == ((B, n, ref.last) if ref.last > 1 else (B, n)), (name, tuple(src.shape))
+            srcs.append(src)
+        m = len(srcs)
+        return ((ctypes.c_void_p * m)(*[self.alloc.ptr(s) for s in srcs]), (ctypes.c_long * m)(*[n for _, n in ref.names]), m, srcs)
 
     def _bind(self, st, P):
         L, A, dt = self.lib, self.alloc, self.dtype
@@ -370,10 +394,20 @@
                     L.call("rd_copy_rows", A.ptr(src), n * b["last"] * 4, self.p(o), row, off * b["last"] * 4,
                            n * b["last"] * 4, B, st_)
                     off += n
+            elif k == "sorted_fg" and isinstance(b["pc"], InputParts):
+                dec = b.get("decode")
+                pp, pn, pm, keep_p = self._parts(b["pc"], din)
+                mp, mn, mm, keep_m = self._parts(b["mask"], din)
+                L.call("rd_sorted_foreground_decode", self.p(b["score"]), self.p(b["delta"]), pp, pn, pm, mp, mn, mm, B, b["N"], b["k"],
+                       b["D"], b["apply_sigmoid"], dec["is_bin"] if dec else 0, self.p(b["out_score"]),
+                       self.p(b["out_delta"]), self.p(b["out_pc"]), A.ptr(b["idx"]) if b["idx"] is not None else None,
+                       self.p(dec["out"]) if dec else None, A.ptr(b["ws"]), b["ws_bytes"], st_)
             elif k == "sorted_fg":
                 L.call("rd_sorted_foreground", self.p(b["score"]), self.p(b["delta"]), self.p(b["pc"]), self.p(b["mask"]),
                        B, b["N"], b["k"], b["D"], b["apply_sigmoid"], self.p(b["out_score"]), self.p(b["out_delta"]),
                        self.p(b["out_pc"]), A.ptr(b["idx"]) if b["idx"] is not None else None, A.ptr(b["ws"]), b["ws_bytes"], st_)
+            elif k == "decode" and b.get("fused") and only is None:
+                pass
             elif k == "decode":
                 L.call("rd_decode3d_bbox", self.p(b["delta"]), self.p(b["pc"]), self.p(b["out"]), B, b["k"],
                        b["box_type"], b["is_bin"], st_)
```

Result: no change. 1022, median of 6 (+0.4%).
